# abiswas-odu/metagenomics

Hardware: NVIDIA B200
Metric: overlap_graph_build_reads_per_sec (higher is better)
Workload: dtype u64

## Files before the change

### include/ogb.h

```cpp
#ifndef OGB_H_
#define OGB_H_

#include <stddef.h>
#include <stdint.h>

#ifdef __cplusplus
extern "C" {
#endif

#define OGB_VERSION 210

enum {
	OGB_OK = 0,
	OGB_E_ARG = 1,
	OGB_E_CUDA = 2,
	OGB_E_NCCL = 3,
	OGB_E_STATE = 4,
	OGB_E_CAPACITY = 5,
	OGB_E_IO = 6,
	OGB_E_NOMEM = 7
};

typedef struct ogb_dataset ogb_dataset;
typedef struct ogb_context ogb_context;

typedef struct ogb_edge {
	uint32_t src;
	uint32_t dst;
	uint16_t offset;
	uint8_t orient;
	uint8_t reserved;
} ogb_edge;

enum {
	OGB_KC_HASH = 0,
	OGB_KC_WINDOW,
	OGB_KC_PROBE,
	OGB_KC_VERIFY,
	OGB_KC_ROWS,
	OGB_KC_MARK1,
	OGB_KC_MARK2,
	OGB_KC_MARKANY,
	OGB_KC_KEEP,
	OGB_KC_EMIT,
	OGB_KC_CONTAIN_WINDOW,
	OGB_KC_CONTAIN_PROBE,
	OGB_KC_CONTAIN_VERIFY,
	OGB_KC_EXCH_INDEX,
	OGB_KC_EXCH_ROWS,
	OGB_KC_EXCH_BITS,
	OGB_KC_EXCH_FINAL,
	OGB_KC_PROBE_VERIFY,
	OGB_KC_COUNT = 20
};

typedef struct ogb_stats {
	uint64_t n_reads;
	uint64_t table_buckets;
	uint64_t table_bytes;
	uint64_t n_contained;
	uint64_t contain_probes;
	uint64_t contain_hits;
	uint64_t overlap_probes;
	uint64_t probe_sectors;
	uint64_t candidates;
	uint64_t edges_pre;
	uint64_t edges_pre_local;
	uint64_t pivot_entries;
	uint64_t active_pivots;
	uint64_t edges_final;
	uint64_t nodes_final;
	uint64_t max_degree;
	uint64_t overflow_reads;
	uint32_t kernel_launches;
	uint32_t probe_launches;
	uint32_t hash_partitions;
	uint32_t hash_build_attempts;
	float ms_pack;
	float ms_hash_build;
	float ms_contain;
	float ms_overlap;
	float ms_exchange_pre;
	float ms_mark;
	float ms_reduce;
	float ms_total;
	float ms_scan_kernel;
	float ms_probe_launch;
	float ms_window_launch;
	float ms_kernel[OGB_KC_COUNT];
	uint32_t n_kernel[OGB_KC_COUNT];
} ogb_stats;

int ogb_version(void);
const char *ogb_last_error(void);


int ogb_dataset_create(ogb_dataset **out);
void ogb_dataset_destroy(ogb_dataset *ds);

int ogb_dataset_add_reads(ogb_dataset *ds, const char *bases, const uint64_t *offsets, uint64_t n);

int ogb_dataset_add_file(ogb_dataset *ds, const char *path);

int ogb_dataset_finalize(ogb_dataset *ds, uint32_t min_overlap);

int ogb_dataset_finalize_device(ogb_dataset *ds, ogb_context *ctx, uint32_t min_overlap);

uint64_t ogb_dataset_n_reads(const ogb_dataset *ds);
uint64_t ogb_dataset_n_unique(const ogb_dataset *ds);
uint64_t ogb_dataset_shortest(const ogb_dataset *ds);
uint64_t ogb_dataset_longest(const ogb_dataset *ds);
uint32_t ogb_dataset_min_overlap(const ogb_dataset *ds);

const uint64_t *ogb_dataset_words(const ogb_dataset *ds, uint64_t *n_words);
const uint64_t *ogb_dataset_word_offsets(const ogb_dataset *ds);
const uint16_t *ogb_dataset_lengths(const ogb_dataset *ds);
const uint32_t *ogb_dataset_frequencies(const ogb_dataset *ds);

int ogb_dataset_get_read(const ogb_dataset *ds, uint64_t id, int strand, char *out, uint32_t cap, uint32_t *len);

int ogb_dataset_find_read(const ogb_dataset *ds, const char *bases, uint32_t len, uint64_t *id);


int ogb_context_create(ogb_context **out, int device);

int ogb_nccl_unique_id(void *out128);
int ogb_context_create_dist(ogb_context **out, int device, int rank, int n_ranks, const void *nccl_uid);
void ogb_context_destroy(ogb_context *ctx);
int ogb_context_rank(const ogb_context *ctx, int *rank, int *n_ranks);

int ogb_reads_upload(ogb_context *ctx, const char *bases, const uint64_t *offsets, uint64_t n);
int ogb_reads_upload_packed(ogb_context *ctx, const uint64_t *words, const uint64_t *word_offsets,
                            const uint16_t *lengths, uint64_t n);
int ogb_reads_upload_dataset(ogb_context *ctx, const ogb_dataset *ds);
int ogb_reads_upload_packed_sharded(ogb_context *ctx, const uint64_t *shard_words, uint64_t n_total, uint32_t read_len);

int ogb_hash_build(ogb_context *ctx, uint32_t min_overlap);

int ogb_hash_lookup(ogb_context *ctx, const char *keys, uint64_t n_keys, uint64_t *out, uint64_t out_cap,
                    uint64_t *out_offsets);
uint64_t ogb_hash_string_length(const ogb_context *ctx);
uint64_t ogb_hash_table_size(const ogb_context *ctx);

int ogb_mark_contained(ogb_context *ctx);
int ogb_super_read_ids(ogb_context *ctx, uint64_t *out, uint64_t cap);

int ogb_mate_lookup(ogb_context *ctx, const char *bases, const uint64_t *offsets, uint64_t n_seqs, uint32_t min_overlap,
                    uint32_t *out_id, uint8_t *out_orient);

int ogb_build_graph(ogb_context *ctx, int keep_pre);

int ogb_graph_edge_count(ogb_context *ctx, int which, uint64_t *n);
int ogb_graph_edges(ogb_context *ctx, int which, ogb_edge *out, uint64_t cap);

int ogb_graph_edges_shard(ogb_context *ctx, ogb_edge *out, uint64_t cap, uint64_t *n_out);
int ogb_graph_checksum(ogb_context *ctx, int which, uint64_t *xor_out, uint64_t *sum_out);


typedef struct ogb_cedge {
	uint32_t src;
	uint32_t dst;
	uint64_t offset;
	uint64_t list_start;
	uint32_t count;
	uint32_t twin;
	uint8_t orient;
	uint8_t reserved[3];
	uint32_t reserved2;
} ogb_cedge;

typedef struct ogb_clist_item {
	uint32_t read;
	uint16_t offset;
	uint8_t orient;
	uint8_t reserved;
} ogb_clist_item;

typedef struct ogb_simplify_stats {
	uint64_t n_edges_in, n_edges_out, n_items;
	uint64_t merges, dead_ends;
	uint32_t iterations;
	uint32_t rounds;
	uint32_t jumps;
	uint32_t launches;
	float ms;
	float ms_setup;
	float ms_sweeps;
	float ms_dead_ends;
	float ms_lists;
	uint32_t reserved;
} ogb_simplify_stats;

int ogb_graph_simplify(ogb_context *ctx, ogb_simplify_stats *stats);
int ogb_graph_composite_edges(ogb_context *ctx, ogb_cedge *edges, uint64_t edge_cap, ogb_clist_item *items, uint64_t item_cap);


typedef struct ogb_unitig {
	uint32_t edge;
	uint32_t src;
	uint32_t dst;
	uint8_t orient;
	uint8_t reserved[3];
	uint64_t length;
	uint64_t start;
} ogb_unitig;

typedef struct ogb_spell_stats {
	uint64_t unitigs;
	uint64_t bases;
	uint64_t words;
	uint32_t launches;
	float ms;
} ogb_spell_stats;

int ogb_graph_spell(ogb_context *ctx, int canonical_only, uint64_t first, uint64_t count, ogb_spell_stats *stats);
int ogb_graph_unitigs(ogb_context *ctx, ogb_unitig *recs, uint64_t rec_cap, void *out, uint64_t out_cap, int ascii);
int ogb_graph_write_unitigs(ogb_context *ctx, const char *path);

int ogb_get_stats(ogb_context *ctx, ogb_stats *out);

int ogb_timer_begin(ogb_context *ctx);
int ogb_timer_end(ogb_context *ctx, float *ms);
int ogb_l2_flush(ogb_context *ctx, size_t bytes);

int ogb_gather_ceiling(ogb_context *ctx, size_t buffer_bytes, uint32_t gather_bytes, double *gb_per_s);

int ogb_alloc_host(void **out, size_t bytes);
void ogb_free_host(void *p);


int ogb_synth_genome(uint64_t seed, uint64_t len, char *out);

int ogb_synth_reads(uint64_t seed, const char *genomes, const uint64_t *g_offsets, const double *weights,
                    uint32_t n_genomes, uint64_t n_reads, uint32_t len_min, uint32_t len_max, int paired,
                    double insert_mean, double insert_sd, char *out_bases, uint64_t out_cap,
                    uint64_t *out_offsets);

#ifdef __cplusplus
}
#endif
#endif
```

### metagenomics_b200/_lib.py

```python
import ctypes as C
import os

_HERE = os.path.dirname(os.path.abspath(__file__))
LIB_PATH = os.environ.get("OGB_LIB") or os.path.join(_HERE, "libogb.so")

OGB_OK, OGB_E_ARG, OGB_E_CUDA, OGB_E_NCCL, OGB_E_STATE, OGB_E_CAPACITY, OGB_E_IO, OGB_E_NOMEM = range(8)


class OgbError(RuntimeError):
    def __init__(self, code, msg):
        super().__init__(f"libogb error {code}: {msg}")
        self.code = code


class Edge(C.Structure):
    _fields_ = [("src", C.c_uint32), ("dst", C.c_uint32), ("offset", C.c_uint16), ("orient", C.c_uint8),
                ("reserved", C.c_uint8)]


class Stats(C.Structure):
    _fields_ = [(n, C.c_uint64) for n in (
        "n_reads", "table_buckets", "table_bytes", "n_contained", "contain_probes", "contain_hits",
        "overlap_probes", "probe_sectors", "candidates", "edges_pre", "edges_pre_local", "pivot_entries",
        "active_pivots", "edges_final", "nodes_final", "max_degree", "overflow_reads")] + [
        ("kernel_launches", C.c_uint32), ("probe_launches", C.c_uint32), ("hash_partitions", C.c_uint32), ("hash_build_attempts", C.c_uint32)] + [(n, C.c_float) for n in (
            "ms_pack", "ms_hash_build", "ms_contain", "ms_overlap", "ms_exchange_pre", "ms_mark", "ms_reduce",
            "ms_total", "ms_scan_kernel", "ms_probe_launch", "ms_window_launch")] + [
        ("ms_kernel", C.c_float * 20), ("n_kernel", C.c_uint32 * 20)]

    KERNEL_CLASSES = ("hash_insert", "window_part", "probe_parts", "verify", "rows_finish", "mark_fast1", "mark_fast2", "mark_any", "keep", "emit",
                      "contain_window", "contain_probe", "contain_verify", "exch_index", "exch_rows", "exch_bits", "exch_final", "probe_verify")

    def as_dict(self):
        d = {n: getattr(self, n) for n, _ in self._fields_ if n not in ("ms_kernel", "n_kernel")}
        d["kernels"] = {k: {"ms": float(self.ms_kernel[i]), "launches": int(self.n_kernel[i])} for i, k in enumerate(self.KERNEL_CLASSES) if self.n_kernel[i]}
        return d


class SimplifyStats(C.Structure):
    _fields_ = [(n, C.c_uint64) for n in ("n_edges_in", "n_edges_out", "n_items", "merges", "dead_ends")] + [
        (n, C.c_uint32) for n in ("iterations", "rounds", "jumps", "launches")] + [
        (n, C.c_float) for n in ("ms", "ms_setup", "ms_sweeps", "ms_dead_ends", "ms_lists")] + [("reserved", C.c_uint32)]

    def as_dict(self):
        return {n: getattr(self, n) for n, _ in self._fields_ if n != "reserved"}


class SpellStats(C.Structure):
    _fields_ = [(n, C.c_uint64) for n in ("unitigs", "bases", "words")] + [("launches", C.c_uint32), ("ms", C.c_float)]

    def as_dict(self):
        return {n: getattr(self, n) for n, _ in self._fields_}


_u64p = C.POINTER(C.c_uint64)
_vp = C.c_void_p
PROTOTYPES = {
    "ogb_version": (C.c_int, []),
    "ogb_last_error": (C.c_char_p, []),
    "ogb_dataset_create": (C.c_int, [C.POINTER(_vp)]),
    "ogb_dataset_destroy": (None, [_vp]),
    "ogb_dataset_add_reads": (C.c_int, [_vp, _vp, _vp, C.c_uint64]),
    "ogb_dataset_add_file": (C.c_int, [_vp, C.c_char_p]),
    "ogb_dataset_finalize": (C.c_int, [_vp, C.c_uint32]),
    "ogb_dataset_finalize_device": (C.c_int, [_vp, _vp, C.c_uint32]),
    "ogb_dataset_n_reads": (C.c_uint64, [_vp]),
    "ogb_dataset_n_unique": (C.c_uint64, [_vp]),
    "ogb_dataset_shortest": (C.c_uint64, [_vp]),
    "ogb_dataset_longest": (C.c_uint64, [_vp]),
    "ogb_dataset_min_overlap": (C.c_uint32, [_vp]),
    "ogb_dataset_words": (_vp, [_vp, _u64p]),
    "ogb_dataset_word_offsets": (_vp, [_vp]),
    "ogb_dataset_lengths": (_vp, [_vp]),
    "ogb_dataset_frequencies": (_vp, [_vp]),
    "ogb_dataset_get_read": (C.c_int, [_vp, C.c_uint64, C.c_int, _vp, C.c_uint32, C.POINTER(C.c_uint32)]),
    "ogb_dataset_find_read": (C.c_int, [_vp, C.c_char_p, C.c_uint32, _u64p]),
    "ogb_context_create": (C.c_int, [C.POINTER(_vp), C.c_int]),
    "ogb_nccl_unique_id": (C.c_int, [_vp]),
    "ogb_context_create_dist": (C.c_int, [C.POINTER(_vp), C.c_int, C.c_int, C.c_int, _vp]),
    "ogb_context_destroy": (None, [_vp]),
    "ogb_context_rank": (C.c_int, [_vp, C.POINTER(C.c_int), C.POINTER(C.c_int)]),
    "ogb_reads_upload": (C.c_int, [_vp, _vp, _vp, C.c_uint64]),
    "ogb_reads_upload_packed": (C.c_int, [_vp, _vp, _vp, _vp, C.c_uint64]),
    "ogb_reads_upload_dataset": (C.c_int, [_vp, _vp]),
    "ogb_reads_upload_packed_sharded": (C.c_int, [_vp, _vp, C.c_uint64, C.c_uint32]),
    "ogb_hash_build": (C.c_int, [_vp, C.c_uint32]),
    "ogb_hash_lookup": (C.c_int, [_vp, _vp, C.c_uint64, _vp, C.c_uint64, _vp]),
    "ogb_hash_string_length": (C.c_uint64, [_vp]),
    "ogb_hash_table_size": (C.c_uint64, [_vp]),
    "ogb_mark_contained": (C.c_int, [_vp]),
    "ogb_super_read_ids": (C.c_int, [_vp, _vp, C.c_uint64]),
    "ogb_mate_lookup": (C.c_int, [_vp, _vp, _vp, C.c_uint64, C.c_uint32, _vp, _vp]),
    "ogb_build_graph": (C.c_int, [_vp, C.c_int]),
    "ogb_graph_edge_count": (C.c_int, [_vp, C.c_int, _u64p]),
    "ogb_graph_edges": (C.c_int, [_vp, C.c_int, _vp, C.c_uint64]),
    "ogb_graph_edges_shard": (C.c_int, [_vp, _vp, C.c_uint64, _u64p]),
    "ogb_graph_checksum": (C.c_int, [_vp, C.c_int, _u64p, _u64p]),
    "ogb_graph_simplify": (C.c_int, [_vp, C.POINTER(SimplifyStats)]),
    "ogb_graph_composite_edges": (C.c_int, [_vp, _vp, C.c_uint64, _vp, C.c_uint64]),
    "ogb_graph_spell": (C.c_int, [_vp, C.c_int, C.c_uint64, C.c_uint64, C.POINTER(SpellStats)]),
    "ogb_graph_unitigs": (C.c_int, [_vp, _vp, C.c_uint64, _vp, C.c_uint64, C.c_int]),
    "ogb_graph_write_unitigs": (C.c_int, [_vp, C.c_char_p]),
    "ogb_get_stats": (C.c_int, [_vp, C.POINTER(Stats)]),
    "ogb_timer_begin": (C.c_int, [_vp]),
    "ogb_timer_end": (C.c_int, [_vp, C.POINTER(C.c_float)]),
    "ogb_l2_flush": (C.c_int, [_vp, C.c_size_t]),
    "ogb_gather_ceiling": (C.c_int, [_vp, C.c_size_t, C.c_uint32, C.POINTER(C.c_double)]),
    "ogb_alloc_host": (C.c_int, [C.POINTER(_vp), C.c_size_t]),
    "ogb_free_host": (None, [_vp]),
    "ogb_synth_genome": (C.c_int, [C.c_uint64, C.c_uint64, _vp]),
    "ogb_synth_reads": (C.c_int, [C.c_uint64, _vp, _vp, _vp, C.c_uint32, C.c_uint64, C.c_uint32, C.c_uint32, C.c_int,
                                  C.c_double, C.c_double, _vp, C.c_uint64, _vp]),
}

_lib = None


def lib():
    global _lib
    if _lib is None:
        if not os.path.exists(LIB_PATH):
            raise OgbError(-1, f"{LIB_PATH} is missing: run `python -c 'import __graft_entry__ as g; g.build()'` "
                               "(there is no CPU fallback)")
        l = C.CDLL(LIB_PATH, mode=C.RTLD_GLOBAL)
        for name, (res, args) in PROTOTYPES.items():
            f = getattr(l, name)
            f.restype, f.argtypes = res, args
        _lib = l
    return _lib


def check(rc):
    if rc != OGB_OK:
        raise OgbError(rc, lib().ogb_last_error().decode("utf-8", "replace"))
```

### metagenomics_b200/csrc/ogb_device.cu

```cuda

#include "ogb_internal.h"
#include "ogb_kernels.cuh"
#include "ogb_contract.cuh"
#include "ogb_spell.cuh"

#include <algorithm>
#include <chrono>
#include <cstdio>
#include <cstring>
#include <dlfcn.h>
#include <string>
#include <vector>

#define CUDA_TRY(x)                                                                                      \
	do {                                                                                                 \
		cudaError_t e_ = (x);                                                                            \
		if (e_ != cudaSuccess) {                                                                         \
			ogb_set_error("CUDA error %s at %s:%d (%s)", cudaGetErrorString(e_), __FILE__, __LINE__, #x); \
			return OGB_E_CUDA;                                                                           \
		}                                                                                                \
	} while (0)
#define OGB_TRY(x) do { int r_ = (x); if (r_ != OGB_OK) return r_; } while (0)

typedef struct ncclComm *ncclComm_t;
typedef struct { char internal[128]; } ncclUniqueId;
enum { NCCL_UINT8 = 1, NCCL_UINT32 = 3, NCCL_UINT64 = 5 };
enum { NCCL_MAX = 2 };
struct NcclApi {
	void *lib = nullptr;
	int (*GetUniqueId)(ncclUniqueId *) = nullptr;
	int (*CommInitRank)(ncclComm_t *, int, ncclUniqueId, int) = nullptr;
	int (*CommDestroy)(ncclComm_t) = nullptr;
	int (*AllGather)(const void *, void *, size_t, int, ncclComm_t, cudaStream_t) = nullptr;
	int (*AllReduce)(const void *, void *, size_t, int, int, ncclComm_t, cudaStream_t) = nullptr;
	int (*Broadcast)(const void *, void *, size_t, int, int, ncclComm_t, cudaStream_t) = nullptr;
	int (*Send)(const void *, size_t, int, int, ncclComm_t, cudaStream_t) = nullptr;
	int (*Recv)(void *, size_t, int, int, ncclComm_t, cudaStream_t) = nullptr;
	int (*GroupStart)() = nullptr;
	int (*GroupEnd)() = nullptr;
	const char *(*GetErrorString)(int) = nullptr;
};
static NcclApi g_nccl;
static int nccl_load()
{
	if (g_nccl.lib) return OGB_OK;
	void *lib = dlopen("libnccl.so.2", RTLD_NOW | RTLD_GLOBAL);
	if (!lib) lib = dlopen("libnccl.so", RTLD_NOW | RTLD_GLOBAL);
	if (!lib) { ogb_set_error("cannot load libnccl.so.2: %s", dlerror()); return OGB_E_NCCL; }
#define SYM(field, name) *(void **)(&g_nccl.field) = dlsym(lib, name); if (!g_nccl.field) { ogb_set_error("libnccl: missing %s", name); return OGB_E_NCCL; }
	SYM(GetUniqueId, "ncclGetUniqueId") SYM(CommInitRank, "ncclCommInitRank") SYM(CommDestroy, "ncclCommDestroy")
	SYM(AllGather, "ncclAllGather") SYM(AllReduce, "ncclAllReduce") SYM(Broadcast, "ncclBroadcast") SYM(Send, "ncclSend") SYM(Recv, "ncclRecv")
	SYM(GroupStart, "ncclGroupStart") SYM(GroupEnd, "ncclGroupEnd") SYM(GetErrorString, "ncclGetErrorString")
#undef SYM
	g_nccl.lib = lib;
	return OGB_OK;
}
#define NCCL_TRY(x)                                                                                   \
	do {                                                                                              \
		int r_ = (x);                                                                                 \
		if (r_ != 0) { ogb_set_error("NCCL error %s at %s:%d", g_nccl.GetErrorString(r_), __FILE__, __LINE__); return OGB_E_NCCL; } \
	} while (0)

template <class T> struct Pool {
	T *p = nullptr;
	size_t cap = 0;
	int ensure(size_t need)
	{
		if (need <= cap) return OGB_OK;
		if (p) cudaFree(p);
		p = nullptr; cap = 0;
		cudaError_t e = cudaMalloc((void **)&p, need * sizeof(T));
		if (e != cudaSuccess) { ogb_set_error("cudaMalloc of %zu bytes failed: %s", need * sizeof(T), cudaGetErrorString(e)); return OGB_E_NOMEM; }
		cap = need;
		return OGB_OK;
	}
	void release() { if (p) cudaFree(p); p = nullptr; cap = 0; }
};

enum { OGB_MAX_RANKS = 64, XCHG_PER_RANK = 8, XCHG_SCRATCH = XCHG_PER_RANK * OGB_MAX_RANKS, XCHG_WORDS = XCHG_SCRATCH + 8 };


template <class T> struct Tmp {
	T *p = nullptr;
	cudaStream_t st = nullptr;
	int ensure(size_t need, cudaStream_t stream)
	{
		if (p) return OGB_OK;
		st = stream;
		cudaError_t e = cudaMallocAsync((void **)&p, std::max<size_t>(need, 1) * sizeof(T), stream);
		if (e != cudaSuccess) { ogb_set_error("cudaMallocAsync of %zu bytes failed: %s", need * sizeof(T), cudaGetErrorString(e)); p = nullptr; return OGB_E_NOMEM; }
		return OGB_OK;
	}
	void release() { if (p) cudaFreeAsync(p, st); p = nullptr; }
};

enum { EV_BEGIN = 0, EV_PACK0, EV_PACK1, EV_HASH0, EV_HASH1, EV_CONT0, EV_CONT1, EV_OVL0, EV_OVL1, EV_XPRE1, EV_MARK1, EV_RED1, EV_K3A, EV_K3B, EV_T0, EV_T1, EV_COUNT };

struct ogb_context {
	int device = 0, rank = 0, nranks = 1, sm_count = 148;
	cudaStream_t stream = nullptr;
	cudaStream_t stream2 = nullptr;
	cudaEvent_t ev_probe[2] = {}, ev_verify[2] = {};
	cudaEvent_t ev_pk[2 * 64] = {};
	cudaEvent_t ev_pm[64] = {};
	u32 n_pk = 0;
	struct KEv { cudaEvent_t a = nullptr, b = nullptr; int cls = 0; };
	std::vector<KEv> kev;
	u32 n_kev = 0;
	ncclComm_t comm = nullptr;
	cudaEvent_t ev[EV_COUNT] = {};
	Pool<u64> words, meta;
	Pool<u64> ds_words;
	ogb_dataset *pending_ds = nullptr;
	Pool<char> stage_bytes;
	Pool<u64> stage_offs;
	Pool<unsigned short> stage_lens;
	u32 n = 0, uniform_len = 0, uniform_pw = 0, min_len = 0, max_len = 0;
	bool have_reads = false;
	uint64_t reads_stamp = 0;
	Pool<u32> slots, summary;
	u32 nb = 0, h = 0, nparts = 1;
	bool use_summary = false;
	bool have_table = false;
	Pool<u64> sup;
	Pool<u32> contained;
	bool contain_done = false, any_contained = false;
	Pool<u64> pos, sums, surv;
	Pool<u64> cand, big;
	Pool<u32> cnt, cntc, scratch_keys;
	Pool<ogb_edge> fin, pre, fin_stage;
	Pool<u64> slots_e, ext;
	Pool<u32> deg;
	Pool<u32> rows, more, more_own, ebits, hrows;
	u64 more_stride = 0, more_cap = 0;
	cudaStream_t xs = nullptr;
	u32 *peer_rows[64] = {};
	const void *rows_shared = nullptr;
	bool rows_dma = false;
	cudaEvent_t ev_rows[2] = {}, ev_xs = nullptr;
	Pool<u32> cand_q, fill, ov_q;
	Pool<u64> cand_v, ov_e;
	u64 cand_cap = 0;
	Pool<u32> pq_b, pq_f, pq_q;
	u64 *d_pq_cursor = nullptr;
	bool partitioned = false, part_chunk_set = false;
	u64 pq_cap = 0;
	u32 pq_slack = 5;
	u64 *d_cursor = nullptr;
	u64 *d_xchg = nullptr;
	u32 slot_cap = 64;
	u32 chunk_reads = 1u << 16;
	int probe_blocks_per_sm = 0, verify_blocks_per_sm = 0;
	Pool<char> flush;
	u64 n_final = 0, n_pre = 0;
	u64 fin_own_off = 0, fin_own_cnt = 0;
	bool have_graph = false, have_pre = false;
	u64 *d_ctr = nullptr, *h_ctr = nullptr;
	u64 *d_tot = nullptr;
	Pool<CEntry> sE;
	Pool<CRec> s_rec;
	Pool<u32> s_rowptr, s_cp, s_info, s_list, s_keep, s_items, s_blocker;
	Pool<uint8_t> s_state, s_ready, s_flag;
	Pool<u64> s_epos, s_lpos, s_ctr;
	Pool<ogb_cedge> s_out;
	Pool<ogb_clist_item> s_out_items;
	bool have_simplified = false;
	uint64_t s_stamp = 0;
	ogb_simplify_stats sst = {};
	Pool<u32> sp_sel, sp_ioff, sp_nw;
	Pool<u64> sp_rank, sp_ipos, sp_wpos, sp_words;
	Pool<ogb_unitig> sp_rec;
	Pool<char> sp_ascii;
	bool have_spelled = false;
	u64 sp_first = 0;
	ogb_spell_stats spst = {};
	const void *l2_window_ptr = nullptr;
	size_t l2_window_bytes = 0;
	bool l2_refused = false;
	ogb_stats st = {};
	u32 launches = 0;

	ReadStore rs() const { ReadStore r; r.words = words.p; r.meta = uniform_len ? nullptr : meta.p; r.n = n; r.uniform_len = uniform_len; r.uniform_pw = uniform_pw; return r; }
	Table tb() const
	{
		Table t;
		t.slots = slots.p; t.summary = use_summary ? summary.p : nullptr; t.nb = nb; t.nparts = nparts; t.part_buckets = nb / nparts;
		t.sub = nparts / nranks; t.my_rank = rank; t.h = h; t.ctr = d_ctr;
		return t;
	}
	void shard(u32 &lo, u32 &hi) const
	{
		u64 per = ((u64)n + nranks - 1) / nranks;
		lo = (u32)std::min<u64>(n, per * rank);
		hi = (u32)std::min<u64>(n, per * (rank + 1));
	}
};

enum { OGB_KEV_MAX = 4096 };
static int kev_begin(ogb_context *c, int cls, cudaStream_t st)
{
	if (c->n_kev >= OGB_KEV_MAX) return -1;
	if (c->n_kev >= c->kev.size()) {
		ogb_context::KEv e;
		if (cudaEventCreate(&e.a) != cudaSuccess || cudaEventCreate(&e.b) != cudaSuccess) { cudaGetLastError(); return -1; }
		c->kev.push_back(e);
	}
	const int i = (int)c->n_kev++;
	c->kev[i].cls = cls;
	cudaEventRecord(c->kev[i].a, st);
	return i;
}
static void kev_end(ogb_context *c, int i, cudaStream_t st) { if (i >= 0) cudaEventRecord(c->kev[i].b, st); }
static void kev_collect(ogb_context *c)
{
	for (u32 i = 0; i < c->n_kev; i++) {
		float ms = 0;
		if (cudaEventElapsedTime(&ms, c->kev[i].a, c->kev[i].b) == cudaSuccess) { c->st.ms_kernel[c->kev[i].cls] += ms; c->st.n_kernel[c->kev[i].cls]++; }
		else cudaGetLastError();
	}
	c->n_kev = 0;
}
#define KEV(cls, stream, launch) do { const int kev_i_ = kev_begin(c, cls, stream); launch; kev_end(c, kev_i_, stream); } while (0)

static int fetch_words_cb(ogb_dataset *ds);

static int ctr_zero(ogb_context *c) { CUDA_TRY(cudaMemsetAsync(c->d_ctr, 0, CTR_COUNT * sizeof(u64), c->stream)); return OGB_OK; }
static int ctr_fetch(ogb_context *c)
{
	CUDA_TRY(cudaMemcpyAsync(c->h_ctr, c->d_ctr, CTR_COUNT * sizeof(u64), cudaMemcpyDeviceToHost, c->stream));
	CUDA_TRY(cudaStreamSynchronize(c->stream));
	return OGB_OK;
}
static int grid_for(ogb_context *c, const void *kernel, int block)
{
	int per_sm = 1;
	if (cudaOccupancyMaxActiveBlocksPerMultiprocessor(&per_sm, kernel, block, 0) != cudaSuccess || per_sm < 1) per_sm = 1;
	return c->sm_count * per_sm;
}
static float ev_ms(ogb_context *c, int a, int b) { float ms = 0; if (cudaEventElapsedTime(&ms, c->ev[a], c->ev[b]) != cudaSuccess) { cudaGetLastError(); return 0; } return ms; }

static int context_create_common(ogb_context **out, int device)
{
	if (!out) { ogb_set_error("ogb_context_create: out is NULL"); return OGB_E_ARG; }
	*out = nullptr;
	int count = 0;
	cudaError_t e = cudaGetDeviceCount(&count);
	if (e != cudaSuccess || count == 0) {
		ogb_set_error("no usable CUDA device (%s); libogb has no CPU fallback", e != cudaSuccess ? cudaGetErrorString(e) : "device count 0");
		cudaGetLastError();
		return OGB_E_CUDA;
	}
	if (device < 0 || device >= count) { ogb_set_error("device %d out of range (%d devices)", device, count); return OGB_E_ARG; }
	CUDA_TRY(cudaSetDevice(device));
	ogb_context *c = new ogb_context();
	c->device = device;
	cudaDeviceProp prop;
	CUDA_TRY(cudaGetDeviceProperties(&prop, device));
	c->sm_count = prop.multiProcessorCount;
	{
		const char *g = getenv("OGB_L2_FETCH");
		size_t gran = g ? (size_t)atoi(g) : 0;
		if (gran == 32 || gran == 64 || gran == 128) cudaDeviceSetLimit(cudaLimitMaxL2FetchGranularity, gran);
		cudaGetLastError();
	}
	CUDA_TRY(cudaStreamCreateWithFlags(&c->stream, cudaStreamNonBlocking));
	{
		cudaMemPool_t pool;
		if (cudaDeviceGetDefaultMemPool(&pool, device) == cudaSuccess) { uint64_t keep = 2ull << 30; cudaMemPoolSetAttribute(pool, cudaMemPoolAttrReleaseThreshold, &keep); }
		cudaGetLastError();
	}
	for (int i = 0; i < EV_COUNT; i++) CUDA_TRY(cudaEventCreate(&c->ev[i]));
	for (int i = 0; i < 128; i++) CUDA_TRY(cudaEventCreate(&c->ev_pk[i]));
	for (int i = 0; i < 64; i++) CUDA_TRY(cudaEventCreate(&c->ev_pm[i]));
	CUDA_TRY(cudaMalloc((void **)&c->d_ctr, CTR_COUNT * sizeof(u64)));
	CUDA_TRY(cudaMalloc((void **)&c->d_tot, 2 * sizeof(u64)));
	CUDA_TRY(cudaMalloc((void **)&c->d_cursor, 2 * sizeof(u64)));
	CUDA_TRY(cudaMalloc((void **)&c->d_pq_cursor, OGB_MAXPART * sizeof(u64)));
	CUDA_TRY(cudaMalloc((void **)&c->d_xchg, XCHG_WORDS * sizeof(u64)));
	CUDA_TRY(cudaMemset(c->d_xchg, 0, XCHG_WORDS * sizeof(u64)));
	CUDA_TRY(cudaStreamCreateWithFlags(&c->stream2, cudaStreamNonBlocking));
	CUDA_TRY(cudaStreamCreateWithFlags(&c->xs, cudaStreamNonBlocking));
	for (int i = 0; i < 2; i++) CUDA_TRY(cudaEventCreateWithFlags(&c->ev_rows[i], cudaEventDisableTiming));
	CUDA_TRY(cudaEventCreateWithFlags(&c->ev_xs, cudaEventDisableTiming));
	for (int i = 0; i < 2; i++) { CUDA_TRY(cudaEventCreateWithFlags(&c->ev_probe[i], cudaEventDisableTiming)); CUDA_TRY(cudaEventCreateWithFlags(&c->ev_verify[i], cudaEventDisableTiming)); }
	CUDA_TRY(cudaMemset(c->d_tot, 0, 2 * sizeof(u64)));
	CUDA_TRY(cudaMallocHost((void **)&c->h_ctr, CTR_COUNT * sizeof(u64)));
	CUDA_TRY(cudaMemset(c->d_ctr, 0, CTR_COUNT * sizeof(u64)));
	*out = c;
	return OGB_OK;
}

extern "C" int ogb_context_create(ogb_context **out, int device) { return context_create_common(out, device); }

extern "C" int ogb_nccl_unique_id(void *out128)
{
	if (!out128) { ogb_set_error("ogb_nccl_unique_id: NULL output"); return OGB_E_ARG; }
	OGB_TRY(nccl_load());
	ncclUniqueId id;
	NCCL_TRY(g_nccl.GetUniqueId(&id));
	memcpy(out128, &id, sizeof id);
	return OGB_OK;
}

extern "C" int ogb_context_create_dist(ogb_context **out, int device, int rank, int n_ranks, const void *nccl_uid)
{
	if (n_ranks < 1 || rank < 0 || rank >= n_ranks) { ogb_set_error("ogb_context_create_dist: bad rank %d of %d", rank, n_ranks); return OGB_E_ARG; }
	if (n_ranks > OGB_MAX_RANKS || n_ranks > OGB_MAXPART) { ogb_set_error("ogb_context_create_dist: at most %d ranks", OGB_MAX_RANKS < OGB_MAXPART ? OGB_MAX_RANKS : OGB_MAXPART); return OGB_E_ARG; }
	OGB_TRY(context_create_common(out, device));
	ogb_context *c = *out;
	c->rank = rank; c->nranks = n_ranks;
	if (n_ranks > 1) {
		if (!nccl_uid) { ogb_set_error("ogb_context_create_dist: NULL nccl id"); return OGB_E_ARG; }
		OGB_TRY(nccl_load());
		ncclUniqueId id;
		memcpy(&id, nccl_uid, sizeof id);
		NCCL_TRY(g_nccl.CommInitRank(&c->comm, n_ranks, id, rank));
	}
	return OGB_OK;
}

extern "C" void ogb_context_destroy(ogb_context *c)
{
	if (!c) return;
	cudaSetDevice(c->device);
	cudaStreamSynchronize(c->stream);
	if (c->pending_ds) fetch_words_cb(c->pending_ds);
	if (c->l2_window_ptr) cudaCtxResetPersistingL2Cache();
	if (c->stream2) cudaStreamSynchronize(c->stream2);
	if (c->xs) cudaStreamSynchronize(c->xs);
	{
		bool mapped = false;
		for (int p = 0; p < 64; p++) if (c->peer_rows[p]) { cudaIpcCloseMemHandle(c->peer_rows[p]); c->peer_rows[p] = nullptr; mapped = true; }
		if (mapped && c->comm) {
			g_nccl.AllReduce(c->d_xchg + XCHG_SCRATCH + 6, c->d_xchg + XCHG_SCRATCH + 6, 1, NCCL_UINT64, 2 , c->comm, c->stream);
			cudaStreamSynchronize(c->stream);
		}
	}
	if (c->comm) g_nccl.CommDestroy(c->comm);
	c->words.release(); c->meta.release(); c->ds_words.release(); c->stage_bytes.release(); c->stage_offs.release(); c->stage_lens.release();
	c->slots.release(); c->summary.release(); c->sup.release(); c->contained.release(); c->pos.release();
	c->sums.release(); c->surv.release(); c->cand.release(); c->big.release(); c->cntc.release(); c->cnt.release();
	c->scratch_keys.release(); c->fin.release(); c->pre.release(); c->flush.release(); c->fin_stage.release();
	c->sE.release(); c->s_rec.release(); c->s_rowptr.release(); c->s_cp.release(); c->s_info.release(); c->s_list.release(); c->s_keep.release(); c->s_items.release(); c->s_blocker.release();
	c->s_state.release(); c->s_ready.release(); c->s_flag.release(); c->s_epos.release(); c->s_lpos.release(); c->s_ctr.release(); c->s_out.release(); c->s_out_items.release();
	c->sp_sel.release(); c->sp_ioff.release(); c->sp_nw.release(); c->sp_rank.release(); c->sp_ipos.release(); c->sp_wpos.release(); c->sp_words.release();
	c->sp_rec.release(); c->sp_ascii.release();
	if (c->d_ctr) cudaFree(c->d_ctr);
	if (c->d_tot) cudaFree(c->d_tot);
	if (c->d_cursor) cudaFree(c->d_cursor);
	if (c->d_pq_cursor) cudaFree(c->d_pq_cursor);
	c->pq_b.release(); c->pq_f.release(); c->pq_q.release();
	if (c->d_xchg) cudaFree(c->d_xchg);
	c->cand_q.release(); c->deg.release(); c->fill.release(); c->ov_q.release();
	c->cand_v.release(); c->slots_e.release(); c->ext.release(); c->ov_e.release(); c->rows.release(); c->more.release(); c->more_own.release(); c->hrows.release(); c->ebits.release();
	if (c->h_ctr) cudaFreeHost(c->h_ctr);
	for (int i = 0; i < EV_COUNT; i++) if (c->ev[i]) cudaEventDestroy(c->ev[i]);
	for (int i = 0; i < 128; i++) if (c->ev_pk[i]) cudaEventDestroy(c->ev_pk[i]);
	for (int i = 0; i < 64; i++) if (c->ev_pm[i]) cudaEventDestroy(c->ev_pm[i]);
	for (auto &e : c->kev) { if (e.a) cudaEventDestroy(e.a); if (e.b) cudaEventDestroy(e.b); }
	for (int i = 0; i < 2; i++) { if (c->ev_probe[i]) cudaEventDestroy(c->ev_probe[i]); if (c->ev_verify[i]) cudaEventDestroy(c->ev_verify[i]); }
	for (int i = 0; i < 2; i++) if (c->ev_rows[i]) cudaEventDestroy(c->ev_rows[i]);
	if (c->ev_xs) cudaEventDestroy(c->ev_xs);
	if (c->xs) cudaStreamDestroy(c->xs);
	if (c->stream2) cudaStreamDestroy(c->stream2);
	if (c->stream) cudaStreamDestroy(c->stream);
	delete c;
}

extern "C" int ogb_context_rank(const ogb_context *c, int *rank, int *n_ranks)
{
	if (!c) { ogb_set_error("NULL context"); return OGB_E_ARG; }
	if (rank) *rank = c->rank;
	if (n_ranks) *n_ranks = c->nranks;
	return OGB_OK;
}

extern "C" int ogb_alloc_host(void **out, size_t bytes)
{
	if (!out) { ogb_set_error("ogb_alloc_host: NULL output"); return OGB_E_ARG; }
	cudaError_t e = cudaMallocHost(out, bytes ? bytes : 1);
	if (e != cudaSuccess) { ogb_set_error("cudaMallocHost(%zu) failed: %s", bytes, cudaGetErrorString(e)); cudaGetLastError(); return OGB_E_CUDA; }
	return OGB_OK;
}
extern "C" void ogb_free_host(void *p) { if (p) cudaFreeHost(p); }


static int layout_reads(ogb_context *c, const std::vector<u32> &lens, u64 &total_words, std::vector<u64> &meta_host)
{
	u32 n = (u32)lens.size();
	u32 mn = 0xFFFFFFFFu, mx = 0;
	for (u32 i = 0; i < n; i++) { mn = std::min(mn, lens[i]); mx = std::max(mx, lens[i]); }
	c->n = n; c->min_len = n ? mn : 0; c->max_len = mx;
	if (n && mn == mx) {
		c->uniform_len = mx;
		c->uniform_pw = ((mx + 63) >> 6) << 1;
		total_words = (u64)n * 2 * c->uniform_pw;
		meta_host.clear();
	} else {
		c->uniform_len = 0; c->uniform_pw = 0;
		meta_host.resize(n);
		u64 off = 0;
		for (u32 i = 0; i < n; i++) {
			if (off >= (1ull << 47)) { ogb_set_error("read store too large"); return OGB_E_CAPACITY; }
			meta_host[i] = (off << 16) | lens[i];
			off += 2 * (u64)(((lens[i] + 63) >> 6) << 1);
		}
		total_words = off;
	}
	return OGB_OK;
}

static int upload_common(ogb_context *c, u64 total_words, const std::vector<u64> &meta_host)
{
	OGB_TRY(c->words.ensure(total_words + 8));
	CUDA_TRY(cudaMemsetAsync(c->words.p + total_words, 0, 8 * sizeof(u64), c->stream));
	if (!meta_host.empty()) {
		OGB_TRY(c->meta.ensure(meta_host.size()));
		CUDA_TRY(cudaMemcpyAsync(c->meta.p, meta_host.data(), meta_host.size() * sizeof(u64), cudaMemcpyHostToDevice, c->stream));
	}
	c->slot_cap = 64;
	c->reads_stamp++;
	c->have_reads = true; c->have_table = false; c->contain_done = false; c->any_contained = false; c->have_graph = false; c->have_pre = false; c->have_spelled = false;
	return OGB_OK;
}

extern "C" int ogb_reads_upload(ogb_context *c, const char *bases, const uint64_t *offsets, uint64_t n)
{
	if (!c || (n && (!bases || !offsets))) { ogb_set_error("ogb_reads_upload: NULL argument"); return OGB_E_ARG; }
	if (n >= (1ull << 30)) { ogb_set_error("ogb_reads_upload: at most 2^30-1 reads per context"); return OGB_E_CAPACITY; }
	CUDA_TRY(cudaSetDevice(c->device));
	std::vector<u32> lens(n);
	for (u64 i = 0; i < n; i++) {
		u64 L = offsets[i + 1] - offsets[i];
		if (L < 2 || L > 65535) { ogb_set_error("ogb_reads_upload: read %llu has length %llu (allowed 2..65535)", (unsigned long long)(i + 1), (unsigned long long)L); return OGB_E_ARG; }
		lens[i] = (u32)L;
	}
	u64 total_words = 0;
	std::vector<u64> meta_host;
	OGB_TRY(layout_reads(c, lens, total_words, meta_host));
	OGB_TRY(upload_common(c, total_words, meta_host));
	if (n == 0) return OGB_OK;
	u64 nbytes = offsets[n] - offsets[0];
	OGB_TRY(c->stage_bytes.ensure(nbytes));
	OGB_TRY(c->stage_offs.ensure(n + 1));
	std::vector<u64> rel(n + 1);
	for (u64 i = 0; i <= n; i++) rel[i] = offsets[i] - offsets[0];
	CUDA_TRY(cudaEventRecord(c->ev[EV_PACK0], c->stream));
	CUDA_TRY(cudaMemcpyAsync(c->stage_bytes.p, bases + offsets[0], nbytes, cudaMemcpyHostToDevice, c->stream));
	CUDA_TRY(cudaMemcpyAsync(c->stage_offs.p, rel.data(), (n + 1) * sizeof(u64), cudaMemcpyHostToDevice, c->stream));
	u32 max_pw = ((c->max_len + 63) >> 6) << 1;
	u64 threads = (u64)n * max_pw;
	k_pack_ascii<<<(unsigned)((threads + 255) / 256), 256, 0, c->stream>>>(c->stage_bytes.p, c->stage_offs.p, c->words.p,
	                                                                      c->uniform_len ? nullptr : c->meta.p, (u32)n, c->uniform_len, c->uniform_pw, max_pw);
	CUDA_TRY(cudaGetLastError());
	CUDA_TRY(cudaEventRecord(c->ev[EV_PACK1], c->stream));
	CUDA_TRY(cudaStreamSynchronize(c->stream));
	c->st.ms_pack = ev_ms(c, EV_PACK0, EV_PACK1);
	c->st.n_reads = n;
	return OGB_OK;
}

extern "C" int ogb_reads_upload_packed(ogb_context *c, const uint64_t *words, const uint64_t *word_offsets, const uint16_t *lengths, uint64_t n)
{
	if (!c || (n && (!words || !word_offsets || !lengths))) { ogb_set_error("ogb_reads_upload_packed: NULL argument"); return OGB_E_ARG; }
	if (n >= (1ull << 30)) { ogb_set_error("ogb_reads_upload_packed: at most 2^30-1 reads per context"); return OGB_E_CAPACITY; }
	CUDA_TRY(cudaSetDevice(c->device));
	uint16_t mn = 0xFFFF, mx = 0;
	for (u64 i = 0; i < n; i++) { mn = std::min(mn, lengths[i]); mx = std::max(mx, lengths[i]); }
	if (n && mn < 2) { ogb_set_error("ogb_reads_upload_packed: a read is shorter than 2"); return OGB_E_ARG; }
	u64 total_words = 0;
	std::vector<u64> meta_host;
	const u64 in_words = n ? word_offsets[n] - word_offsets[0] : 0;
	const bool regular = n && mn == mx && in_words == n * (u64)((mx + 31) / 32);
	if (regular) {
		c->n = (u32)n; c->min_len = c->max_len = mx; c->uniform_len = mx; c->uniform_pw = ((mx + 63) >> 6) << 1;
		total_words = n * 2 * c->uniform_pw;
	} else {
		std::vector<u32> lens(n);
		for (u64 i = 0; i < n; i++) lens[i] = lengths[i];
		OGB_TRY(layout_reads(c, lens, total_words, meta_host));
	}
	OGB_TRY(upload_common(c, total_words, meta_host));
	if (n == 0) return OGB_OK;
	OGB_TRY(c->stage_bytes.ensure(in_words * sizeof(u64)));
	std::vector<u64> rel;
	const u64 *offs_src = (const u64 *)word_offsets;
	if (!regular) {
		OGB_TRY(c->stage_offs.ensure(n + 1));
		OGB_TRY(c->stage_lens.ensure(n));
		if (word_offsets[0] != 0) { rel.resize(n + 1); for (u64 i = 0; i <= n; i++) rel[i] = word_offsets[i] - word_offsets[0]; offs_src = rel.data(); }
	}
	CUDA_TRY(cudaEventRecord(c->ev[EV_PACK0], c->stream));
	CUDA_TRY(cudaMemcpyAsync(c->stage_bytes.p, words + word_offsets[0], in_words * sizeof(u64), cudaMemcpyHostToDevice, c->stream));
	if (!regular) {
		CUDA_TRY(cudaMemcpyAsync(c->stage_offs.p, offs_src, (n + 1) * sizeof(u64), cudaMemcpyHostToDevice, c->stream));
		CUDA_TRY(cudaMemcpyAsync(c->stage_lens.p, lengths, n * sizeof(uint16_t), cudaMemcpyHostToDevice, c->stream));
	}
	u32 max_pw = ((c->max_len + 63) >> 6) << 1;
	u64 threads = (u64)n * max_pw;
	k_pack_words<<<(unsigned)((threads + 255) / 256), 256, 0, c->stream>>>((const u64 *)c->stage_bytes.p, regular ? nullptr : c->stage_offs.p,
	                                                                      regular ? nullptr : c->stage_lens.p, c->words.p,
	                                                                      c->uniform_len ? nullptr : c->meta.p, (u32)n, c->uniform_len, c->uniform_pw, max_pw);
	CUDA_TRY(cudaGetLastError());
	CUDA_TRY(cudaEventRecord(c->ev[EV_PACK1], c->stream));
	CUDA_TRY(cudaStreamSynchronize(c->stream));
	c->st.ms_pack = ev_ms(c, EV_PACK0, EV_PACK1);
	c->st.n_reads = n;
	return OGB_OK;
}

extern "C" int ogb_reads_upload_dataset(ogb_context *c, const ogb_dataset *ds)
{
	if (!c || !ds) { ogb_set_error("ogb_reads_upload_dataset: NULL argument"); return OGB_E_ARG; }
	if (ds->resident_ctx == c && ds->resident_stamp == c->reads_stamp && c->have_reads) return OGB_OK;
	uint64_t nw = 0;
	const uint64_t *w = ogb_dataset_words(ds, &nw);
	return ogb_reads_upload_packed(c, w, ogb_dataset_word_offsets(ds), ogb_dataset_lengths(ds), ogb_dataset_n_unique(ds));
}

extern "C" int ogb_reads_upload_packed_sharded(ogb_context *c, const uint64_t *shard_words, uint64_t n_total, uint32_t read_len)
{
	if (!c || (n_total && !shard_words)) { ogb_set_error("ogb_reads_upload_packed_sharded: NULL argument"); return OGB_E_ARG; }
	if (n_total >= (1ull << 30)) { ogb_set_error("ogb_reads_upload_packed_sharded: at most 2^30-1 reads per context"); return OGB_E_CAPACITY; }
	if (read_len < 2 || read_len > 65535) { ogb_set_error("ogb_reads_upload_packed_sharded: read length %u (allowed 2..65535)", read_len); return OGB_E_ARG; }
	CUDA_TRY(cudaSetDevice(c->device));
	const int G = c->nranks;
	c->n = (u32)n_total; c->min_len = c->max_len = read_len; c->uniform_len = read_len; c->uniform_pw = ((read_len + 63) >> 6) << 1;
	const u64 per = (n_total + G - 1) / G, stride = 2ull * c->uniform_pw, nw = (read_len + 31) / 32;
	const u64 total_words = per * G * stride;
	std::vector<u64> none;
	OGB_TRY(upload_common(c, total_words, none));
	if (n_total == 0) return OGB_OK;
	u32 lo, hi;
	c->shard(lo, hi);
	const u64 nloc = hi - lo;
	OGB_TRY(c->stage_bytes.ensure(std::max<u64>(nloc * nw, 1) * sizeof(u64)));
	CUDA_TRY(cudaEventRecord(c->ev[EV_PACK0], c->stream));
	if (nloc) {
		CUDA_TRY(cudaMemcpyAsync(c->stage_bytes.p, shard_words, nloc * nw * sizeof(u64), cudaMemcpyHostToDevice, c->stream));
		const u64 threads = nloc * c->uniform_pw;
		k_pack_words<<<(unsigned)((threads + 255) / 256), 256, 0, c->stream>>>((const u64 *)c->stage_bytes.p, nullptr, nullptr, c->words.p + (u64)lo * stride, nullptr,
		                                                                      (u32)nloc, c->uniform_len, c->uniform_pw, c->uniform_pw);
		CUDA_TRY(cudaGetLastError());
	}
	if (G > 1) NCCL_TRY(g_nccl.AllGather(c->words.p + per * stride * c->rank, c->words.p, per * stride, NCCL_UINT64, c->comm, c->stream));
	CUDA_TRY(cudaEventRecord(c->ev[EV_PACK1], c->stream));
	CUDA_TRY(cudaStreamSynchronize(c->stream));
	c->st.ms_pack = ev_ms(c, EV_PACK0, EV_PACK1);
	c->st.n_reads = n_total;
	return OGB_OK;
}

static int exclusive_scan(ogb_context *c, const u32 *cnt, u32 n, u64 *out, u64 *d_total, u64 *d_max = nullptr, u64 *d_more = nullptr);

static int fetch_words_cb(ogb_dataset *ds)
{
	ogb_context *c = (ogb_context *)ds->fetch_ctx;
	ds->fetch = nullptr; ds->fetch_ctx = nullptr;
	if (!c) return OGB_OK;
	if (c->pending_ds == ds) c->pending_ds = nullptr;
	CUDA_TRY(cudaSetDevice(c->device));
	ds->words.resize(ds->pending_words);
	if (ds->pending_words) {
		CUDA_TRY(cudaMemcpyAsync(ds->words.data(), c->ds_words.p, ds->pending_words * sizeof(u64), cudaMemcpyDeviceToHost, c->stream));
		CUDA_TRY(cudaStreamSynchronize(c->stream));
	}
	ds->pending_words = 0;
// ... 227 lines not shown
		c->partitioned = e ? atoi(e) != 0 : true;
	}
	c->launches = 0;
	c->n_kev = 0;
	memset(c->st.ms_kernel, 0, sizeof c->st.ms_kernel); memset(c->st.n_kernel, 0, sizeof c->st.n_kernel);
	CUDA_TRY(cudaEventRecord(c->ev[EV_HASH0], c->stream));
	u64 sub_limit = OGB_MAXPART / c->nranks, nb = 0;
	bool k1_direct = false;
	for (int attempt = 0;; attempt++) {
		if (attempt == 12) { ogb_set_error("ogb_hash_build: a hash partition kept filling up (%u partitions, %.1f buckets per read)", c->nparts, buckets_per_read); return OGB_E_CAPACITY; }
		nb = std::max<u64>((u64)(buckets_per_read * c->n) + 1, 512);
		{
			const u64 slice_bytes = nb * OGB_BWORDS * sizeof(u32) / c->nranks;
			u64 sub = slice_bytes > (192ull << 20) ? (slice_bytes + (160ull << 20) - 1) / (160ull << 20) : 1;
			const char *e = getenv("OGB_SUB_PARTITIONS");
			if (e && atoi(e) >= 1) sub = (u64)atoi(e);
			sub = std::max<u64>(1, std::min<u64>(sub, sub_limit));
			c->nparts = (u32)(c->nranks * sub);
		}
		nb = (nb + c->nparts - 1) / c->nparts * c->nparts;
		if (nb >= (1ull << 32)) { ogb_set_error("index too large"); return OGB_E_CAPACITY; }
		c->nb = (u32)nb;
		OGB_TRY(c->slots.ensure(nb * OGB_BWORDS));
		if (c->use_summary) OGB_TRY(c->summary.ensure(nb));
		{
			const u64 pb = nb / c->nranks;
			CUDA_TRY(cudaMemsetAsync(c->slots.p + pb * OGB_BWORDS * c->rank, 0, pb * OGB_BWORDS * sizeof(u32), c->stream));
			if (c->use_summary) CUDA_TRY(cudaMemsetAsync(c->summary.p + pb * c->rank, 0, pb * sizeof(u32), c->stream));
		}
		CUDA_TRY(cudaMemsetAsync(c->d_ctr + CTR_TABLE_FULL, 0, sizeof(u64), c->stream));
		if (c->n) {
			u64 threads = (u64)c->n * 4;
			const u32 sub = c->nparts / c->nranks;
			const char *eq = getenv("OGB_K1_QUEUES");
			const bool queued = sub > 1 && !k1_direct && !(eq && atoi(eq) == 0);
			if (queued) {
				const u64 qcap = threads / c->nparts * 5 / 4 + 4096;
				OGB_TRY(c->pq_b.ensure(qcap * sub)); OGB_TRY(c->pq_f.ensure(qcap * sub)); OGB_TRY(c->pq_q.ensure(qcap * sub));
				KeyQueue kq;
				kq.b = c->pq_b.p; kq.f = c->pq_f.p; kq.v = c->pq_q.p; kq.cursor = c->d_pq_cursor; kq.cap = qcap;
				kq.nparts = c->nparts; kq.first = (u32)c->rank * sub; kq.count = sub;
				CUDA_TRY(cudaMemsetAsync(c->d_pq_cursor, 0, OGB_MAXPART * sizeof(u64), c->stream));
				const u64 tiles = (threads + 256 * OGB_KPT - 1) / (256 * OGB_KPT);
				const int ke = kev_begin(c, OGB_KC_HASH, c->stream);
				k_key_part<<<(unsigned)std::min<u64>(grid_for(c, (const void *)k_key_part, 256), tiles), 256, 0, c->stream>>>(c->rs(), c->tb(), kq);
				k_insert_parts<<<grid_for(c, (const void *)k_insert_parts, 256), 256, 0, c->stream>>>(c->tb(), kq);
				kev_end(c, ke, c->stream);
				CUDA_TRY(cudaGetLastError());
				c->launches += 2;
			}
			if (!queued) {
				KEV(OGB_KC_HASH, c->stream, (k_hash_insert<<<(unsigned)((threads + 255) / 256), 256, 0, c->stream>>>(c->rs(), c->tb())));
				CUDA_TRY(cudaGetLastError());
				c->launches++;
			}
		}
		u64 full = 0;
		if (c->nranks > 1) NCCL_TRY(g_nccl.AllReduce(c->d_ctr + CTR_TABLE_FULL, c->d_ctr + CTR_TABLE_FULL, 1, NCCL_UINT64, NCCL_MAX, c->comm, c->stream));
		CUDA_TRY(cudaMemcpyAsync(c->h_ctr + CTR_TABLE_FULL, c->d_ctr + CTR_TABLE_FULL, sizeof(u64), cudaMemcpyDeviceToHost, c->stream));
		if (c->nranks > 1) {
			const u64 pb = nb / c->nranks;
			const int ke = kev_begin(c, OGB_KC_EXCH_INDEX, c->stream);
			NCCL_TRY(g_nccl.AllGather(c->slots.p + pb * OGB_BWORDS * c->rank, c->slots.p, pb * OGB_BWORDS, NCCL_UINT32, c->comm, c->stream));
			if (c->use_summary) NCCL_TRY(g_nccl.AllGather(c->summary.p + pb * c->rank, c->summary.p, pb, NCCL_UINT32, c->comm, c->stream));
			kev_end(c, ke, c->stream);
		}
		CUDA_TRY(cudaEventRecord(c->ev[EV_HASH1], c->stream));
		CUDA_TRY(cudaStreamSynchronize(c->stream));
		kev_collect(c);
		full = c->h_ctr[CTR_TABLE_FULL];
		c->st.hash_build_attempts = (uint32_t)attempt + 1;
		if (!full) break;
		if (full >= 2 && !k1_direct) { k1_direct = true; continue; }
		if (c->nparts > (u32)c->nranks) sub_limit = std::max<u64>(1, c->nparts / c->nranks / 2);
		else buckets_per_read *= 2;
	}
	OGB_TRY(l2_keep_summary(c, true));
	c->st.ms_hash_build = ev_ms(c, EV_HASH0, EV_HASH1);
	c->st.table_buckets = nb;
	c->st.hash_partitions = c->nparts;
	c->st.table_bytes = nb * OGB_BWORDS * sizeof(u32);
	c->part_chunk_set = false; c->pq_slack = 5;
	if (!c->partitioned && c->chunk_reads > (1u << 16)) c->chunk_reads = 1u << 16;
	c->have_table = true; c->contain_done = false; c->any_contained = false; c->have_graph = false;
	c->st.ms_contain = 0; c->st.n_contained = 0; c->st.contain_probes = 0; c->st.contain_hits = 0;
	return OGB_OK;
}

extern "C" uint64_t ogb_hash_string_length(const ogb_context *c) { return c ? c->h : 0; }
extern "C" uint64_t ogb_hash_table_size(const ogb_context *c) { return c ? (uint64_t)c->nb * OGB_SLOTS : 0; }

extern "C" int ogb_hash_lookup(ogb_context *c, const char *keys, uint64_t n_keys, uint64_t *out, uint64_t out_cap, uint64_t *out_offsets)
{
	if (!c || !out_offsets || (n_keys && !keys)) { ogb_set_error("ogb_hash_lookup: NULL argument"); return OGB_E_ARG; }
	if (!c->have_table) { ogb_set_error("ogb_hash_lookup: build the hash table first"); return OGB_E_STATE; }
	CUDA_TRY(cudaSetDevice(c->device));
	const u32 h = c->h, kw = (h + 31) / 32;
	out_offsets[0] = 0;
	if (n_keys == 0) return OGB_OK;
	std::vector<u64> packed(n_keys * (kw + 2) + 4, 0);
	for (u64 k = 0; k < n_keys; k++)
		for (u32 i = 0; i < h; i++) {
			u64 code;
			switch (keys[k * h + i]) {
			case 'A': case 'a': code = 0; break;
			case 'C': case 'c': code = 1; break;
			case 'G': case 'g': code = 2; break;
			case 'T': case 't': code = 3; break;
			default: ogb_set_error("ogb_hash_lookup: key %llu is not ACGT", (unsigned long long)k); return OGB_E_ARG;
			}
			packed[k * (kw + 2) + (i >> 5)] |= code << (62 - 2 * (i & 31));
		}
	Pool<u64> d_keys, d_pos, d_out;
	Pool<u32> d_cnt;
	int rc = OGB_OK;
	std::vector<u32> cnt(n_keys);
	std::vector<u64> pos(n_keys + 1, 0);
	auto run = [&]() -> int {
		OGB_TRY(d_keys.ensure(packed.size())); OGB_TRY(d_cnt.ensure(n_keys)); OGB_TRY(d_pos.ensure(n_keys + 1));
		CUDA_TRY(cudaMemcpyAsync(d_keys.p, packed.data(), packed.size() * sizeof(u64), cudaMemcpyHostToDevice, c->stream));
		unsigned grid = (unsigned)((n_keys + 127) / 128);
		k_lookup<<<grid, 128, 0, c->stream>>>(c->rs(), c->tb(), d_keys.p, kw, n_keys, d_cnt.p, nullptr, nullptr, 0);
		CUDA_TRY(cudaGetLastError());
		CUDA_TRY(cudaMemcpyAsync(cnt.data(), d_cnt.p, n_keys * sizeof(u32), cudaMemcpyDeviceToHost, c->stream));
		CUDA_TRY(cudaStreamSynchronize(c->stream));
		for (u64 k = 0; k < n_keys; k++) pos[k + 1] = pos[k] + cnt[k];
		for (u64 k = 0; k <= n_keys; k++) out_offsets[k] = pos[k];
		if (pos[n_keys] > out_cap || (pos[n_keys] && !out)) { ogb_set_error("ogb_hash_lookup: output needs %llu entries", (unsigned long long)pos[n_keys]); return OGB_E_CAPACITY; }
		if (pos[n_keys] == 0) return OGB_OK;
		OGB_TRY(d_out.ensure(pos[n_keys]));
		CUDA_TRY(cudaMemcpyAsync(d_pos.p, pos.data(), (n_keys + 1) * sizeof(u64), cudaMemcpyHostToDevice, c->stream));
		k_lookup<<<grid, 128, 0, c->stream>>>(c->rs(), c->tb(), d_keys.p, kw, n_keys, d_cnt.p, d_pos.p, d_out.p, 1);
		CUDA_TRY(cudaGetLastError());
		CUDA_TRY(cudaMemcpyAsync(out, d_out.p, pos[n_keys] * sizeof(u64), cudaMemcpyDeviceToHost, c->stream));
		CUDA_TRY(cudaStreamSynchronize(c->stream));
		for (u64 k = 0; k < n_keys; k++)
			std::sort(out + pos[k], out + pos[k + 1], [](u64 a, u64 b) {
				u64 ia = a & 0x3FFFFFFFFFFFFFFFull, ib = b & 0x3FFFFFFFFFFFFFFFull;
				return ia != ib ? ia < ib : (a >> 62) < (b >> 62);
			});
		return OGB_OK;
	};
	rc = run();
	d_keys.release(); d_pos.release(); d_out.release(); d_cnt.release();
	return rc;
}

static ScanArgs scan_args(ogb_context *c, u32 lo, u32 hi)
{
	ScanArgs a;
	a.R = c->rs(); a.T = c->tb(); a.lo = lo; a.hi = hi;
	a.contained = c->any_contained ? c->contained.p : nullptr;
	a.cand_q = c->cand_q.p; a.cand_v = c->cand_v.p; a.cand_cap = c->cand_cap; a.cand_cursor = c->d_cursor;
	a.sup = c->sup.p; a.slots_e = c->slots_e.p; a.slot_lo = lo; a.cap = c->slot_cap; a.deg = c->deg.p;
	a.ov_q = c->ov_q.p; a.ov_e = c->ov_e.p; a.ov_cap = c->ov_q.cap; a.ctr = c->d_ctr; a.prefetch = 1;
	return a;
}

static GraphView graph_view(const ogb_context *c, u32 lo);

static int share_rows(ogb_context *c)
{
	const int G = c->nranks;
	if (G == 1 || c->rows_shared == (const void *)c->rows.p) return OGB_OK;
	for (int p = 0; p < G; p++) if (c->peer_rows[p]) { cudaIpcCloseMemHandle(c->peer_rows[p]); c->peer_rows[p] = nullptr; }
	c->rows_dma = false;
	c->rows_shared = c->rows.p;
	const char *e = getenv("OGB_ROWS_NCCL");
	u64 ok = !(e && atoi(e) != 0);
	cudaIpcMemHandle_t mine;
	memset(&mine, 0, sizeof mine);
	if (ok && cudaIpcGetMemHandle(&mine, c->rows.p) != cudaSuccess) { cudaGetLastError(); ok = 0; }
	static_assert(sizeof(cudaIpcMemHandle_t) == 64, "IPC handle size");
	const size_t rec = 72;
	Pool<unsigned char> buf;
	OGB_TRY(buf.ensure(rec * G));
	std::vector<unsigned char> host(rec * G, 0);
	memcpy(host.data() + rec * c->rank, &mine, 64);
	memcpy(host.data() + rec * c->rank + 64, &ok, 8);
	CUDA_TRY(cudaMemcpyAsync(buf.p + rec * c->rank, host.data() + rec * c->rank, rec, cudaMemcpyHostToDevice, c->stream));
	NCCL_TRY(g_nccl.AllGather(buf.p + rec * c->rank, buf.p, rec, NCCL_UINT8, c->comm, c->stream));
	CUDA_TRY(cudaMemcpyAsync(host.data(), buf.p, rec * G, cudaMemcpyDeviceToHost, c->stream));
	CUDA_TRY(cudaStreamSynchronize(c->stream));
	buf.release();
	bool all = true;
	for (int p = 0; p < G; p++) { u64 f; memcpy(&f, host.data() + rec * p + 64, 8); all = all && f != 0; }
	u64 opened = all;
	if (all)
		for (int p = 0; p < G && opened; p++) {
			if (p == c->rank) continue;
			cudaIpcMemHandle_t h;
			memcpy(&h, host.data() + rec * p, 64);
			void *ptr = nullptr;
			if (cudaIpcOpenMemHandle(&ptr, h, cudaIpcMemLazyEnablePeerAccess) != cudaSuccess) { cudaGetLastError(); opened = 0; break; }
			c->peer_rows[p] = (u32 *)ptr;
		}
	CUDA_TRY(cudaMemcpyAsync(c->d_xchg + XCHG_SCRATCH + 6, &opened, sizeof(u64), cudaMemcpyHostToDevice, c->stream));
	NCCL_TRY(g_nccl.AllReduce(c->d_xchg + XCHG_SCRATCH + 6, c->d_xchg + XCHG_SCRATCH + 6, 1, NCCL_UINT64, 3 , c->comm, c->stream));
	CUDA_TRY(cudaMemcpyAsync(&opened, c->d_xchg + XCHG_SCRATCH + 6, sizeof(u64), cudaMemcpyDeviceToHost, c->stream));
	CUDA_TRY(cudaStreamSynchronize(c->stream));
	c->rows_dma = opened != 0;
	if (!c->rows_dma) for (int p = 0; p < G; p++) if (c->peer_rows[p]) { cudaIpcCloseMemHandle(c->peer_rows[p]); c->peer_rows[p] = nullptr; }
	return OGB_OK;
}

static int exchange_chunk_rows(ogb_context *c, u32 ci, cudaStream_t st)
{
	const int G = c->nranks;
	const u64 per = ((u64)c->n + G - 1) / G;
	auto range = [&](int r, u64 &a, u64 &b) {
		const u64 lo = std::min<u64>(c->n, per * r), hi = std::min<u64>(c->n, per * (r + 1));
		a = std::min(hi, lo + (u64)ci * c->chunk_reads); b = std::min(hi, a + c->chunk_reads);
	};
	u64 ma, mb;
	range(c->rank, ma, mb);
	if (c->rows_dma) {
		for (int k = 1; k < G && mb > ma; k++) {
			const int p = (c->rank + k) % G;
			CUDA_TRY(cudaMemcpyAsync(c->peer_rows[p] + ma * OGB_ROW_W, c->rows.p + ma * OGB_ROW_W, (mb - ma) * OGB_ROW_W * sizeof(u32), cudaMemcpyDeviceToDevice, st));
		}
		return OGB_OK;
	}
	NCCL_TRY(g_nccl.GroupStart());
	for (int p = 0; p < G; p++) {
		if (p == c->rank) continue;
		u64 pa, pb;
		range(p, pa, pb);
		if (mb > ma) NCCL_TRY(g_nccl.Send(c->rows.p + ma * OGB_ROW_W, (mb - ma) * OGB_ROW_W, NCCL_UINT32, p, c->comm, st));
		if (pb > pa) NCCL_TRY(g_nccl.Recv(c->rows.p + pa * OGB_ROW_W, (pb - pa) * OGB_ROW_W, NCCL_UINT32, p, c->comm, st));
	}
	NCCL_TRY(g_nccl.GroupEnd());
	return OGB_OK;
}

template <int MODE> static int scan_chunks(ogb_context *c, u32 lo, u32 hi)
{
	const bool part_mode = c->partitioned && hi > lo;
	const u32 nwin_u = (c->uniform_len ? c->uniform_len : c->max_len) - c->h - 1;
	{
		const char *e = getenv("OGB_CHUNK_READS");
		if (e && atoll(e) >= 256 && !part_mode) c->chunk_reads = (u32)std::min<long long>(atoll(e), 1ll << 16);
	}
	if (part_mode) {
		if (!c->part_chunk_set) { const char *e = getenv("OGB_CHUNK_READS"); c->chunk_reads = e && atoll(e) >= 256 ? (u32)std::min<long long>(atoll(e), 1ll << 23) : 3u << 17; c->part_chunk_set = true; }
		c->chunk_reads = (u32)std::max<u64>(256, std::min<u64>(c->chunk_reads, (64ull << 20) / std::max<u32>(nwin_u, 1)));
		const u64 pcap = std::min<u64>(c->chunk_reads, hi - lo) * nwin_u / c->nparts * std::min<u64>(c->pq_slack, 4ull * c->nparts) / 4 + 4096;
		OGB_TRY(c->pq_b.ensure(pcap * c->nparts)); OGB_TRY(c->pq_f.ensure(pcap * c->nparts)); OGB_TRY(c->pq_q.ensure(pcap * c->nparts));
		c->pq_cap = pcap;
	} else
	if (c->chunk_reads > (1u << 16)) c->chunk_reads = 1u << 16;
	{
		const u64 want = part_mode ? std::max<u64>(32ull << 20, (u64)c->chunk_reads * 40) : 8ull << 20;
		if (c->cand_cap < want) { OGB_TRY(c->cand_q.ensure(2 * want)); OGB_TRY(c->cand_v.ensure(2 * want)); c->cand_cap = want; }
	}
	int gp = grid_for(c, (const void *)k_probe<MODE>, 256), gv = grid_for(c, (const void *)k_verify<MODE>, 256);
	int gu = grid_for(c, (const void *)k_probe_uniform<MODE>, 256);
	{
		const char *ep = getenv("OGB_PROBE_BLOCKS_PER_SM"), *ev = getenv("OGB_VERIFY_BLOCKS_PER_SM");
		const int bp = ep ? atoi(ep) : c->probe_blocks_per_sm, bv = ev ? atoi(ev) : c->verify_blocks_per_sm;
		if (bp > 0) { gp = std::min(gp, c->sm_count * bp); gu = std::min(gu, c->sm_count * bp); }
		if (bv > 0) gv = std::min(gv, c->sm_count * bv);
	}
	const bool overlap_streams = getenv("OGB_ONE_STREAM") == nullptr;
	cudaStream_t sv = overlap_streams ? c->stream2 : c->stream;
	ScanArgs a = scan_args(c, lo, hi);
	u32 i = 0;
	const bool xchg = MODE == MODE_OVERLAP && c->nranks > 1;
	const u64 per_rank = ((u64)c->n + c->nranks - 1) / c->nranks;
	const u32 n_chunks = (u32)(((xchg ? per_rank : (u64)(hi - lo)) + c->chunk_reads - 1) / c->chunk_reads);
	const GraphView gv_rows = graph_view(c, lo);
	const int g_rows = grid_for(c, (const void *)k_rows_finish<false>, 256);
	const bool fused = part_mode && getenv("OGB_FUSED") && atoi(getenv("OGB_FUSED")) == 1;
	bool have_prev = false;
	ScanArgs a_prev = a;
	u32 prev_i = 0;
	auto finish_chunk = [&](const ScanArgs &av, u32 ci, cudaStream_t after) -> int {
		if (MODE != MODE_OVERLAP) return OGB_OK;
		CUDA_TRY(cudaEventRecord(c->ev_rows[ci & 1], after));
		CUDA_TRY(cudaStreamWaitEvent(c->xs, c->ev_rows[ci & 1], 0));
		KEV(OGB_KC_ROWS, c->xs, (k_rows_finish<false><<<std::min<int>(g_rows, (int)((av.hi - av.lo + 255) / 256)), 256, 0, c->xs>>>(gv_rows, av.lo, av.hi, c->more_own.p, c->more_cap, c->d_ctr, nullptr, 0)));
		c->launches++;
		if (xchg) {
			const int ke = kev_begin(c, OGB_KC_EXCH_ROWS, c->xs);
			OGB_TRY(exchange_chunk_rows(c, ci, c->xs));
			kev_end(c, ke, c->xs);
		}
		return OGB_OK;
	};
	auto flush_prev = [&]() -> int {
		if (!have_prev) return OGB_OK;
		KEV(MODE == MODE_OVERLAP ? OGB_KC_VERIFY : OGB_KC_CONTAIN_VERIFY, c->stream, (k_verify<MODE><<<gv, 256, 0, c->stream>>>(a_prev)));
		c->launches++;
		have_prev = false;
		return finish_chunk(a_prev, prev_i, c->stream);
	};
	for (; i < n_chunks; i++) {
		const u64 b0 = (u64)lo + (u64)i * c->chunk_reads;
		const int q = i & 1;
		if (b0 >= hi) {
			if (fused) OGB_TRY(flush_prev());
			if (xchg) { const int ke = kev_begin(c, OGB_KC_EXCH_ROWS, c->xs); OGB_TRY(exchange_chunk_rows(c, i, c->xs)); kev_end(c, ke, c->xs); }
			continue;
		}
		if (fused) {
			a.lo = (u32)b0; a.hi = (u32)std::min<u64>(hi, b0 + c->chunk_reads);
			a.cand_q = c->cand_q.p + q * c->cand_cap; a.cand_v = c->cand_v.p + q * c->cand_cap; a.cand_cursor = c->d_cursor + q;
			a.prefetch = 0;
			CUDA_TRY(cudaMemsetAsync(a.cand_cursor, 0, sizeof(u64), c->stream));
			CUDA_TRY(cudaMemsetAsync(c->d_pq_cursor, 0, OGB_MAXPART * sizeof(u64), c->stream));
			PartQueue pq;
			pq.b = c->pq_b.p; pq.f = c->pq_f.p; pq.q = c->pq_q.p; pq.cursor = c->d_pq_cursor; pq.cap = c->pq_cap; pq.nparts = c->nparts;
			const u32 nreads = a.hi - a.lo;
			const u64 tiles = ((u64)nreads * nwin_u + 256 * OGB_WPT - 1) / (256 * OGB_WPT);
			const bool uni = c->uniform_len && !a.contained;
			const int gw = grid_for(c, uni ? (const void *)k_window_part<MODE, true> : (const void *)k_window_part<MODE, false>, 256);
			const int kc = MODE == MODE_OVERLAP ? 0 : OGB_KC_CONTAIN_WINDOW - OGB_KC_WINDOW;
			const bool timed = MODE == MODE_OVERLAP && i < 64;
			if (timed) CUDA_TRY(cudaEventRecord(c->ev_pk[2 * i], c->stream));
			if (uni) KEV(OGB_KC_WINDOW + kc, c->stream, (k_window_part<MODE, true><<<(unsigned)std::min<u64>(gw, tiles), 256, 0, c->stream>>>(a, nwin_u, ~0ull / nwin_u + 1, pq)));
			else KEV(OGB_KC_WINDOW + kc, c->stream, (k_window_part<MODE, false><<<(unsigned)std::min<u64>(gw, tiles), 256, 0, c->stream>>>(a, nwin_u, ~0ull / nwin_u + 1, pq)));
			if (timed) CUDA_TRY(cudaEventRecord(c->ev_pm[i], c->stream));
			if (have_prev) {
				KEV(MODE == MODE_OVERLAP ? OGB_KC_PROBE_VERIFY : OGB_KC_CONTAIN_PROBE, c->stream,
				    (k_probe_verify<MODE><<<grid_for(c, (const void *)k_probe_verify<MODE>, 256), 256, 0, c->stream>>>(a, pq, a_prev)));
				OGB_TRY(finish_chunk(a_prev, prev_i, c->stream));
			} else
				KEV(OGB_KC_PROBE + kc, c->stream, (k_probe_parts<MODE><<<grid_for(c, (const void *)k_probe_parts<MODE>, 256), 256, 0, c->stream>>>(a, pq)));
			if (timed) { CUDA_TRY(cudaEventRecord(c->ev_pk[2 * i + 1], c->stream)); c->n_pk = i + 1; }
			c->launches += 2;
			have_prev = true; a_prev = a; prev_i = i;
			continue;
		}
		a.lo = (u32)b0; a.hi = (u32)std::min<u64>(hi, b0 + c->chunk_reads);
		a.cand_q = c->cand_q.p + q * c->cand_cap; a.cand_v = c->cand_v.p + q * c->cand_cap; a.cand_cursor = c->d_cursor + q;
		if (overlap_streams && i >= 2) CUDA_TRY(cudaStreamWaitEvent(c->stream, c->ev_verify[q], 0));
		CUDA_TRY(cudaMemsetAsync(a.cand_cursor, 0, sizeof(u64), c->stream));
		const u32 warps = a.hi - a.lo;
		const bool timed = MODE == MODE_OVERLAP && i < 64;
		if (timed) CUDA_TRY(cudaEventRecord(c->ev_pk[2 * i], c->stream));
		if (part_mode) {
			PartQueue pq;
			pq.b = c->pq_b.p; pq.f = c->pq_f.p; pq.q = c->pq_q.p; pq.cursor = c->d_pq_cursor; pq.cap = c->pq_cap; pq.nparts = c->nparts;
			a.prefetch = 0;
			CUDA_TRY(cudaMemsetAsync(c->d_pq_cursor, 0, OGB_MAXPART * sizeof(u64), c->stream));
			const u64 tiles = ((u64)warps * nwin_u + 256 * OGB_WPT - 1) / (256 * OGB_WPT);
			const bool uni = c->uniform_len && !a.contained;
			const int gw = grid_for(c, uni ? (const void *)k_window_part<MODE, true> : (const void *)k_window_part<MODE, false>, 256), gb = grid_for(c, (const void *)k_probe_parts<MODE>, 256);
			const int kc = MODE == MODE_OVERLAP ? 0 : OGB_KC_CONTAIN_WINDOW - OGB_KC_WINDOW;
			if (uni) KEV(OGB_KC_WINDOW + kc, c->stream, (k_window_part<MODE, true><<<(unsigned)std::min<u64>(gw, tiles), 256, 0, c->stream>>>(a, nwin_u, ~0ull / nwin_u + 1, pq)));
			else KEV(OGB_KC_WINDOW + kc, c->stream, (k_window_part<MODE, false><<<(unsigned)std::min<u64>(gw, tiles), 256, 0, c->stream>>>(a, nwin_u, ~0ull / nwin_u + 1, pq)));
			if (timed) CUDA_TRY(cudaEventRecord(c->ev_pm[i], c->stream));
			KEV(OGB_KC_PROBE + kc, c->stream, (k_probe_parts<MODE><<<gb, 256, 0, c->stream>>>(a, pq)));
			c->launches++;
		} else if (c->uniform_len && !a.contained) {
			const u32 nwin = c->uniform_len - c->h - 1;
			const u64 rounds = ((u64)warps * nwin + 31) / 32;
			KEV(MODE == MODE_OVERLAP ? OGB_KC_PROBE : OGB_KC_CONTAIN_PROBE, c->stream, (k_probe_uniform<MODE><<<(unsigned)std::min<u64>(gu, (rounds * 32 + 255) / 256), 256, 0, c->stream>>>(a, nwin, ~0ull / nwin + 1)));
		} else
			KEV(MODE == MODE_OVERLAP ? OGB_KC_PROBE : OGB_KC_CONTAIN_PROBE, c->stream, (k_probe<MODE><<<(unsigned)std::min<u64>(gp, ((u64)warps * 32 + 255) / 256), 256, 0, c->stream>>>(a)));
		if (timed) { CUDA_TRY(cudaEventRecord(c->ev_pk[2 * i + 1], c->stream)); c->n_pk = i + 1; }
		if (overlap_streams) {
			CUDA_TRY(cudaEventRecord(c->ev_probe[q], c->stream));
			CUDA_TRY(cudaStreamWaitEvent(sv, c->ev_probe[q], 0));
		}
		KEV(MODE == MODE_OVERLAP ? OGB_KC_VERIFY : OGB_KC_CONTAIN_VERIFY, sv, (k_verify<MODE><<<gv, 256, 0, sv>>>(a)));
		if (MODE == MODE_OVERLAP) {
			CUDA_TRY(cudaEventRecord(c->ev_rows[q], sv));
			CUDA_TRY(cudaStreamWaitEvent(c->xs, c->ev_rows[q], 0));
			KEV(OGB_KC_ROWS, c->xs, (k_rows_finish<false><<<std::min<int>(g_rows, (int)((a.hi - a.lo + 255) / 256)), 256, 0, c->xs>>>(gv_rows, a.lo, a.hi, c->more_own.p, c->more_cap, c->d_ctr, nullptr, 0)));
			c->launches++;
			if (xchg) {
				const int ke = kev_begin(c, OGB_KC_EXCH_ROWS, c->xs);
				OGB_TRY(exchange_chunk_rows(c, i, c->xs));
				kev_end(c, ke, c->xs);
			}
		}
		if (overlap_streams) CUDA_TRY(cudaEventRecord(c->ev_verify[q], sv));
		c->launches += 2;
	}
	if (fused) OGB_TRY(flush_prev());
	if (overlap_streams && !fused)
		for (int q = 0; q < 2 && q < (int)i; q++) CUDA_TRY(cudaStreamWaitEvent(c->stream, c->ev_verify[q], 0));
	if (MODE == MODE_OVERLAP) { CUDA_TRY(cudaEventRecord(c->ev_xs, c->xs)); CUDA_TRY(cudaStreamWaitEvent(c->stream, c->ev_xs, 0)); }
	CUDA_TRY(cudaGetLastError());
	return OGB_OK;
}

extern "C" int ogb_mark_contained(ogb_context *c)
{
	if (!c) { ogb_set_error("NULL context"); return OGB_E_ARG; }
	if (!c->have_table) { ogb_set_error("ogb_mark_contained: build the hash table first"); return OGB_E_STATE; }
	CUDA_TRY(cudaSetDevice(c->device));
	OGB_TRY(l2_keep_summary(c, true));
	c->contain_done = true; c->any_contained = false; c->have_graph = false;
	c->st.n_contained = 0; c->st.contain_probes = 0; c->st.contain_hits = 0; c->st.ms_contain = 0;
	OGB_TRY(c->sup.ensure((size_t)c->n + 1));
	CUDA_TRY(cudaMemsetAsync(c->sup.p, 0, ((size_t)c->n + 1) * sizeof(u64), c->stream));
	if (c->n == 0 || c->min_len == c->max_len) { CUDA_TRY(cudaStreamSynchronize(c->stream)); return OGB_OK; }
	OGB_TRY(c->contained.ensure(((size_t)c->n + 31) / 32 + 1));
	u32 lo, hi;
	c->shard(lo, hi);
	CUDA_TRY(cudaEventRecord(c->ev[EV_CONT0], c->stream));
	for (int attempt = 0;; attempt++) {
		if (attempt == 12) { ogb_set_error("ogb_mark_contained: candidate queue kept overflowing"); return OGB_E_CAPACITY; }
		OGB_TRY(ctr_zero(c));
		CUDA_TRY(cudaMemsetAsync(c->sup.p, 0, ((size_t)c->n + 1) * sizeof(u64), c->stream));
		bool saved = c->any_contained;
		c->any_contained = false;
		int rc = scan_chunks<MODE_CONTAIN>(c, lo, hi);
		c->any_contained = saved;
		OGB_TRY(rc);
		OGB_TRY(ctr_fetch(c));
		if (c->h_ctr[CTR_CAND_MAX] > c->cand_cap) { c->chunk_reads = std::max<u32>(256, c->chunk_reads / 2); continue; }
		break;
	}
	c->st.contain_probes = c->h_ctr[CTR_PROBES];
	c->st.contain_hits = c->h_ctr[CTR_CONTAIN_HITS];
	OGB_TRY(ctr_zero(c));
	if (c->nranks > 1) NCCL_TRY(g_nccl.AllReduce(c->sup.p, c->sup.p, c->n, NCCL_UINT64, NCCL_MAX, c->comm, c->stream));
	k_contained_bitmap<<<(c->n + 255) / 256, 256, 0, c->stream>>>(c->sup.p, c->n, c->contained.p, c->d_ctr);
	CUDA_TRY(cudaGetLastError());
	c->launches++;
	CUDA_TRY(cudaEventRecord(c->ev[EV_CONT1], c->stream));
	OGB_TRY(ctr_fetch(c));
	kev_collect(c);
	c->st.ms_contain = ev_ms(c, EV_CONT0, EV_CONT1);
	c->st.n_contained = c->h_ctr[CTR_N_CONTAINED];
	c->any_contained = c->st.n_contained > 0;
	return OGB_OK;
}

extern "C" int ogb_super_read_ids(ogb_context *c, uint64_t *out, uint64_t cap)
{
	if (!c || !out) { ogb_set_error("ogb_super_read_ids: NULL argument"); return OGB_E_ARG; }
	if (cap < (uint64_t)c->n + 1) { ogb_set_error("ogb_super_read_ids: need %u entries", c->n + 1); return OGB_E_CAPACITY; }
	out[0] = 0;
	if (!c->contain_done || c->n == 0) { for (u32 i = 1; i <= c->n; i++) out[i] = 0; return OGB_OK; }
	CUDA_TRY(cudaSetDevice(c->device));
	CUDA_TRY(cudaMemcpyAsync(out + 1, c->sup.p, (size_t)c->n * sizeof(u64), cudaMemcpyDeviceToHost, c->stream));
	CUDA_TRY(cudaStreamSynchronize(c->stream));
	for (u32 i = 1; i <= c->n; i++) out[i] = out[i] ? (uint64_t)(0xFFFFFFFFu - (u32)(out[i] & 0xFFFFFFFFull)) + 1 : 0;
	return OGB_OK;
}

static int exclusive_scan(ogb_context *c, const u32 *cnt, u32 n, u64 *out, u64 *d_total, u64 *d_max, u64 *d_more)
{
	u32 nblocks = (n + OGB_SCAN_ITEMS - 1) / OGB_SCAN_ITEMS;
	if (nblocks == 0) nblocks = 1;
	OGB_TRY(c->sums.ensure(nblocks + 1));
	k_scan_sums<<<nblocks, 256, 0, c->stream>>>(cnt, n, c->sums.p, d_max, d_more);
	k_scan_top<<<1, 1024, 0, c->stream>>>(c->sums.p, nblocks, d_total);
	k_scan_apply<<<nblocks, 256, 0, c->stream>>>(cnt, n, c->sums.p, out);
	CUDA_TRY(cudaGetLastError());
	c->launches += 3;
	return OGB_OK;
}

static GraphView graph_view(const ogb_context *c, u32 lo)
{
	GraphView g;
	const u64 per = ((u64)c->n + c->nranks - 1) / c->nranks;
	g.slots = c->slots_e.p; g.deg = c->deg.p; g.ext = c->ext.p; g.lo = lo; g.cap = c->slot_cap;
	g.rows = c->rows.p; g.more = c->nranks > 1 ? c->more.p : c->more_own.p; g.ebits = c->ebits.p;
	g.more_stride = c->more_stride; g.nrows = per * c->nranks;
	g.per_magic = c->nranks > 1 && per > 1 ? ~0ull / per + 1 : 0;
	g.my_rank = (u32)c->rank;
	return g;
}

template <class T> static int gather_segments(ogb_context *c, Pool<T> &stage, u64 stride, const std::vector<u64> &count, T *out)
{
	const int G = c->nranks;
	if (stride) NCCL_TRY(g_nccl.AllGather(stage.p + stride * c->rank, stage.p, stride * sizeof(T), NCCL_UINT8, c->comm, c->stream));
	u64 at = 0;
	for (int r = 0; r < G; r++) {
		if (count[r]) CUDA_TRY(cudaMemcpyAsync(out + at, stage.p + stride * r, count[r] * sizeof(T), cudaMemcpyDeviceToDevice, c->stream));
		at += count[r];
	}
	return OGB_OK;
}

extern "C" int ogb_build_graph(ogb_context *c, int keep_pre)
{
	if (!c) { ogb_set_error("NULL context"); return OGB_E_ARG; }
	if (!c->have_table) { ogb_set_error("ogb_build_graph: build the hash table first"); return OGB_E_STATE; }
	CUDA_TRY(cudaSetDevice(c->device));
	OGB_TRY(l2_keep_summary(c, true));
	if (!c->contain_done) OGB_TRY(ogb_mark_contained(c));
	c->have_graph = false; c->have_pre = false; c->have_simplified = false; c->have_spelled = false; c->n_final = 0; c->n_pre = 0;
	const u32 n = c->n;
	if (n == 0) { c->have_graph = true; c->have_pre = keep_pre != 0; c->st.edges_pre = c->st.edges_pre_local = c->st.edges_final = c->st.nodes_final = 0; return OGB_OK; }
	u32 lo, hi;
	c->shard(lo, hi);
	const int G = c->nranks;
	const u64 per = ((u64)n + G - 1) / G;
	const u32 nloc = hi - lo;
	{
		const char *e = getenv("OGB_SLOT_CAP");
		if (e && atoi(e) >= 8 && atoi(e) <= 256) c->slot_cap = (u32)atoi(e);
	}
	OGB_TRY(c->cnt.ensure(per + 1));
	OGB_TRY(c->cntc.ensure(per + 1));
	OGB_TRY(c->pos.ensure(per + 1));
	OGB_TRY(c->fill.ensure(per + 1));
	OGB_TRY(c->surv.ensure((per + 1) * OGB_SURV));
	OGB_TRY(c->cand.ensure((per + 1) * OGB_SURV * 2));
	if (G > 1 && per * G * OGB_ROW_W + 64 > c->rows.cap && c->rows_shared) {
		for (int p = 0; p < G; p++) if (c->peer_rows[p]) { cudaIpcCloseMemHandle(c->peer_rows[p]); c->peer_rows[p] = nullptr; }
		c->rows_dma = false; c->rows_shared = nullptr;
		NCCL_TRY(g_nccl.AllReduce(c->d_xchg + XCHG_SCRATCH + 6, c->d_xchg + XCHG_SCRATCH + 6, 1, NCCL_UINT64, 2 , c->comm, c->stream));
		CUDA_TRY(cudaStreamSynchronize(c->stream));
	}
	OGB_TRY(c->rows.ensure(per * G * OGB_ROW_W + 64));
	OGB_TRY(share_rows(c));
	if (c->ov_q.cap == 0) { OGB_TRY(c->ov_q.ensure(1 << 20)); OGB_TRY(c->ov_e.ensure(1 << 20)); }

	CUDA_TRY(cudaEventRecord(c->ev[EV_OVL0], c->stream));
	u64 local_edges = 0, exact_edges = 0, more_need = 0, heavy_max = 0;
	std::vector<u64> seg_cnt(G, 0), hrow_cnt(G, 0);
	for (int attempt = 0;; attempt++) {
		if (attempt == 16) { ogb_set_error("ogb_build_graph: staging pools kept overflowing"); return OGB_E_CAPACITY; }
		OGB_TRY(c->slots_e.ensure(per * c->slot_cap + 64));
		OGB_TRY(c->deg.ensure((size_t)n + 1));
		OGB_TRY(c->ext.ensure(1 << 16));
		if (c->more_cap == 0) c->more_cap = per * 8 + 1024;
		OGB_TRY(c->more_own.ensure((c->more_cap + 1023) & ~1023ull));
		OGB_TRY(ctr_zero(c));
		if (nloc) CUDA_TRY(cudaMemsetAsync(c->deg.p + lo, 0, (size_t)nloc * sizeof(u32), c->stream));
		CUDA_TRY(cudaEventRecord(c->ev[EV_K3A], c->stream));
		OGB_TRY(scan_chunks<MODE_OVERLAP>(c, lo, hi));
		CUDA_TRY(cudaEventRecord(c->ev[EV_K3B], c->stream));
		OGB_TRY(exclusive_scan(c, c->deg.p + lo, nloc, c->pos.p, c->d_tot, c->d_ctr + CTR_MAX_DEGREE, c->d_ctr + CTR_MORE_NEED));
		CUDA_TRY(cudaMemcpyAsync(&local_edges, c->d_tot, sizeof(u64), cudaMemcpyDeviceToHost, c->stream));
		OGB_TRY(ctr_fetch(c));
		const u64 n_over = c->h_ctr[CTR_OVERFLOW], n_heavy = c->h_ctr[CTR_BIG_NODES];
		u64 verdict[XCHG_PER_RANK] = {c->h_ctr[CTR_CAND_MAX] > c->cand_cap, n_over, c->h_ctr[CTR_MAX_DEGREE], local_edges, n_over + n_heavy * c->slot_cap, c->h_ctr[CTR_PQ_OVERFLOW] != 0, c->h_ctr[CTR_MORE_NEED], n_heavy};
		more_need = verdict[6]; heavy_max = n_heavy;
		seg_cnt[0] = local_edges; exact_edges = local_edges;
		hrow_cnt.assign(G, 0); hrow_cnt[0] = n_heavy;
		if (G > 1) {
			CUDA_TRY(cudaMemcpyAsync(c->d_xchg + XCHG_PER_RANK * c->rank, verdict, sizeof verdict, cudaMemcpyHostToDevice, c->stream));
			NCCL_TRY(g_nccl.AllGather(c->d_xchg + XCHG_PER_RANK * c->rank, c->d_xchg, XCHG_PER_RANK, NCCL_UINT64, c->comm, c->stream));
			std::vector<u64> all((size_t)XCHG_PER_RANK * G);
			CUDA_TRY(cudaMemcpyAsync(all.data(), c->d_xchg, all.size() * sizeof(u64), cudaMemcpyDeviceToHost, c->stream));
			CUDA_TRY(cudaStreamSynchronize(c->stream));
			exact_edges = 0;
			for (int r = 0; r < G; r++) {
				const u64 *v = &all[(size_t)XCHG_PER_RANK * r];
				verdict[0] = std::max(verdict[0], v[0]); verdict[1] = std::max(verdict[1], v[1]); verdict[2] = std::max(verdict[2], v[2]); verdict[5] = std::max(verdict[5], v[5]);
				more_need = std::max(more_need, v[6]); heavy_max = std::max(heavy_max, v[7]);
				seg_cnt[r] = v[3]; exact_edges += v[3]; hrow_cnt[r] = v[7];
			}
		}
		if (verdict[5]) { c->pq_slack *= 2; continue; }
		if (more_need > c->more_cap) { c->more_cap = more_need + more_need / 8 + 1024; continue; }
		if (verdict[0]) { c->chunk_reads = std::max<u32>(256, c->chunk_reads / 2); continue; }
		if (verdict[1] > c->ov_q.cap) {
			if (c->slot_cap < 256) c->slot_cap *= 2;
			else { OGB_TRY(c->ov_q.ensure(verdict[1] + verdict[1] / 8 + 1024)); OGB_TRY(c->ov_e.ensure(verdict[1] + verdict[1] / 8 + 1024)); }
			continue;
		}
		c->st.max_degree = verdict[2];
		c->st.overflow_reads = n_heavy;
		if (verdict[1]) {
			OGB_TRY(c->ext.ensure(n_over + n_heavy * c->slot_cap + 64));
			if (n_over) {
				k_heavy_move<<<(nloc + 255) / 256, 256, 0, c->stream>>>(c->slots_e.p, c->deg.p, lo, hi, c->slot_cap, c->ext.p, c->ext.cap, c->fill.p, c->d_ctr);
				k_heavy_place<<<(unsigned)((n_over + 255) / 256), 256, 0, c->stream>>>(c->ov_q.p, c->ov_e.p, n_over, c->slots_e.p, lo, c->slot_cap, c->ext.p, c->fill.p);
				CUDA_TRY(cudaGetLastError());
				c->launches += 2;
			}
		}
		break;
	}
	c->st.overlap_probes = c->h_ctr[CTR_PROBES];
	c->st.probe_sectors = c->h_ctr[CTR_SECTORS];
	c->st.candidates = c->h_ctr[CTR_CANDIDATES];
	c->st.edges_pre_local = local_edges;
	c->st.edges_pre = exact_edges;
	c->n_pre = exact_edges;
	CUDA_TRY(cudaEventRecord(c->ev[EV_OVL1], c->stream));
	OGB_TRY(l2_keep_summary(c, false));

	if (more_need >= (1ull << 32) - 2048) { ogb_set_error("ogb_build_graph: adjacency overflow area too large"); return OGB_E_CAPACITY; }
	c->more_stride = G > 1 ? std::max<u64>(1024, (more_need + 1023) & ~1023ull) : ((c->more_cap + 1023) & ~1023ull);
	if (G > 1) OGB_TRY(c->more.ensure(c->more_stride * G));
	const u64 nrows = per * G, obit_words = c->more_stride / 32;
	OGB_TRY(c->ebits.ensure(nrows + obit_words * G + 2));
	CUDA_TRY(cudaMemsetAsync(c->ebits.p + nrows + obit_words * c->rank, 0, obit_words * sizeof(u32), c->stream));
	if (heavy_max) {
		const u64 hstride = heavy_max;
		if (G > 1) OGB_TRY(c->hrows.ensure(hstride * G * OGB_HROW_W));
		u32 *my_h = G > 1 ? c->hrows.p + hstride * c->rank * OGB_HROW_W : nullptr;
		if (nloc && hrow_cnt[c->rank])
			KEV(OGB_KC_ROWS, c->stream, (k_rows_finish<true><<<grid_for(c, (const void *)k_rows_finish<true>, 256), 256, 0, c->stream>>>(graph_view(c, lo), lo, hi, c->more_own.p, c->more_cap, c->d_ctr, my_h, hstride)));
		CUDA_TRY(cudaGetLastError());
		c->launches++;
		if (G > 1) {
			const int ke = kev_begin(c, OGB_KC_EXCH_ROWS, c->stream);
			NCCL_TRY(g_nccl.AllGather(c->hrows.p + hstride * c->rank * OGB_HROW_W, c->hrows.p, hstride * OGB_HROW_W, NCCL_UINT32, c->comm, c->stream));
			kev_end(c, ke, c->stream);
			OGB_TRY(c->sums.ensure(G + 8));
			CUDA_TRY(cudaMemcpyAsync(c->sums.p, hrow_cnt.data(), (size_t)G * sizeof(u64), cudaMemcpyHostToDevice, c->stream));
			k_scatter_hrows<<<c->sm_count, 256, 0, c->stream>>>(c->hrows.p, hstride, c->sums.p, (u32)G, (u32)c->rank, c->rows.p);
			CUDA_TRY(cudaGetLastError());
			c->launches++;
		}
	}
	if (G > 1 && more_need) {
		const int ke = kev_begin(c, OGB_KC_EXCH_ROWS, c->stream);
		NCCL_TRY(g_nccl.AllGather(c->more_own.p, c->more.p, c->more_stride, NCCL_UINT32, c->comm, c->stream));
		kev_end(c, ke, c->stream);
	}
	CUDA_TRY(cudaEventRecord(c->ev[EV_XPRE1], c->stream));

	const u32 cap_now = c->slot_cap;
	const int g_emit = grid_for(c, (const void *)k_emit<false>, OGB_WARPS * 32);
	if (keep_pre) {
		OGB_TRY(c->pre.ensure(std::max<u64>(exact_edges, 1)));
		if (G == 1) {
			k_emit<true><<<g_emit, OGB_WARPS * 32, 0, c->stream>>>(c->slots_e.p, c->ext.p, c->deg.p, nullptr, c->pos.p, c->pre.p, lo, hi, cap_now, 0, 0);
			CUDA_TRY(cudaGetLastError());
		} else {
			u64 stride = 0;
			for (int r = 0; r < G; r++) stride = std::max(stride, seg_cnt[r]);
			stride = (stride + 63) & ~63ull;
			OGB_TRY(c->fin_stage.ensure(std::max<u64>(stride * G, 1)));
			k_emit<true><<<g_emit, OGB_WARPS * 32, 0, c->stream>>>(c->slots_e.p, c->ext.p, c->deg.p, nullptr, c->pos.p, c->fin_stage.p, lo, hi, cap_now, stride * c->rank, 0);
			CUDA_TRY(cudaGetLastError());
			OGB_TRY(gather_segments(c, c->fin_stage, stride, seg_cnt, c->pre.p));
		}
		c->have_pre = true;
	}

	MarkArgs m;
	m.G = graph_view(c, lo);
	m.hi = hi; m.cnt = c->cnt.p; m.cntc = c->cntc.p; m.cand = c->cand.p;
	OGB_TRY(c->big.ensure((local_edges + 1) * 3));
	m.big = c->big.p; m.big_cap = local_edges + 1;
	if (c->scratch_keys.cap == 0) OGB_TRY(c->scratch_keys.ensure(1 << 20));
	for (int attempt = 0;; attempt++) {
		if (attempt == 4) { ogb_set_error("ogb_build_graph: neighbour-set scratch kept overflowing"); return OGB_E_CAPACITY; }
		OGB_TRY(ctr_zero(c));
		m.scratch_keys = c->scratch_keys.p; m.scratch_cap = c->scratch_keys.cap; m.ctr = c->d_ctr;
		KEV(OGB_KC_MARK1, c->stream, (k_mark_fast<1><<<grid_for(c, (const void *)k_mark_fast<1>, OGB_WARPS * 32), OGB_WARPS * 32, 0, c->stream>>>(m)));
		if (c->st.max_degree > 32) KEV(OGB_KC_MARK2, c->stream, (k_mark_fast<2><<<grid_for(c, (const void *)k_mark_fast<2>, OGB_WARPS * 32), OGB_WARPS * 32, 0, c->stream>>>(m)));
		c->launches += c->st.max_degree > 32 ? 2 : 1;
		KEV(OGB_KC_MARKANY, c->stream, (k_mark_any<<<grid_for(c, (const void *)k_mark_any, OGB_WARPS * 32), OGB_WARPS * 32, 0, c->stream>>>(m)));
		CUDA_TRY(cudaGetLastError());
		c->launches++;
		if (c->st.max_degree * 2 <= OGB_SETCAP) break;
		OGB_TRY(ctr_fetch(c));
		if (c->h_ctr[CTR_SCRATCH_FAIL] == 0) break;
		u64 need = c->h_ctr[CTR_SCRATCH_CURSOR] + 1024;
		OGB_TRY(c->scratch_keys.ensure(need));
	}
	CUDA_TRY(cudaEventRecord(c->ev[EV_MARK1], c->stream));
	if (G > 1) {
		const int ke = kev_begin(c, OGB_KC_EXCH_BITS, c->stream);
		NCCL_TRY(g_nccl.AllGather(c->ebits.p + per * c->rank, c->ebits.p, per, NCCL_UINT32, c->comm, c->stream));
		if (more_need) NCCL_TRY(g_nccl.AllGather(c->ebits.p + nrows + obit_words * c->rank, c->ebits.p + nrows, obit_words, NCCL_UINT32, c->comm, c->stream));
		kev_end(c, ke, c->stream);
	}

	const int ke_keep = kev_begin(c, OGB_KC_KEEP, c->stream);
	if (nloc) k_keep<<<(nloc + 255) / 256, 256, 0, c->stream>>>(m, c->surv.p);
	k_keep_big<<<c->sm_count, 256, 0, c->stream>>>(m);
	kev_end(c, ke_keep, c->stream);
	const int ke_emit = kev_begin(c, OGB_KC_EMIT, c->stream);
	CUDA_TRY(cudaGetLastError());
	c->launches += 2;
	OGB_TRY(exclusive_scan(c, c->cnt.p, nloc, c->pos.p, c->d_tot + 1));
	if (G == 1) {
		OGB_TRY(c->fin.ensure(std::max<u64>(exact_edges, 1)));
		if (nloc) k_emit_small<<<(nloc + 255) / 256, 256, 0, c->stream>>>(c->surv.p, c->cnt.p, c->cntc.p, c->pos.p, c->fin.p, lo, hi, 0);
		k_emit<false><<<g_emit, OGB_WARPS * 32, 0, c->stream>>>(c->slots_e.p, c->ext.p, c->deg.p, c->cntc.p, c->pos.p, c->fin.p, lo, hi, cap_now, 0, OGB_SURV);
		CUDA_TRY(cudaGetLastError());
		kev_end(c, ke_emit, c->stream);
		c->launches += 2;
		u64 tot = 0;
		CUDA_TRY(cudaMemcpyAsync(&tot, c->d_tot + 1, sizeof(u64), cudaMemcpyDeviceToHost, c->stream));
		OGB_TRY(ctr_fetch(c));
		c->n_final = tot; c->fin_own_off = 0; c->fin_own_cnt = tot;
	} else {
		std::vector<u64> fin_cnt(G, 0), all(G, 0);
		CUDA_TRY(cudaMemcpyAsync(c->d_xchg + c->rank, c->d_tot + 1, sizeof(u64), cudaMemcpyDeviceToDevice, c->stream));
		NCCL_TRY(g_nccl.AllGather(c->d_xchg + c->rank, c->d_xchg, 1, NCCL_UINT64, c->comm, c->stream));
		CUDA_TRY(cudaMemcpyAsync(fin_cnt.data(), c->d_xchg, (size_t)G * sizeof(u64), cudaMemcpyDeviceToHost, c->stream));
		CUDA_TRY(cudaStreamSynchronize(c->stream));
		u64 stride = 0, total = 0;
		for (int r = 0; r < G; r++) { stride = std::max(stride, fin_cnt[r]); total += fin_cnt[r]; }
		stride = (stride + 63) & ~63ull;
		c->n_final = total; c->fin_own_off = 0; for (int r = 0; r < c->rank; r++) c->fin_own_off += fin_cnt[r]; c->fin_own_cnt = fin_cnt[c->rank];
		OGB_TRY(c->fin_stage.ensure(std::max<u64>(stride * G, 1)));
		OGB_TRY(c->fin.ensure(std::max<u64>(total, 1)));
		if (nloc) k_emit_small<<<(nloc + 255) / 256, 256, 0, c->stream>>>(c->surv.p, c->cnt.p, c->cntc.p, c->pos.p, c->fin_stage.p, lo, hi, stride * c->rank);
		k_emit<false><<<g_emit, OGB_WARPS * 32, 0, c->stream>>>(c->slots_e.p, c->ext.p, c->deg.p, c->cntc.p, c->pos.p, c->fin_stage.p, lo, hi, cap_now, stride * c->rank, OGB_SURV);
		CUDA_TRY(cudaGetLastError());
		kev_end(c, ke_emit, c->stream);
		c->launches += 2;
		const int ke_fin = kev_begin(c, OGB_KC_EXCH_FINAL, c->stream);
		OGB_TRY(gather_segments(c, c->fin_stage, stride, fin_cnt, c->fin.p));
		kev_end(c, ke_fin, c->stream);
		NCCL_TRY(g_nccl.AllReduce(c->d_ctr + CTR_NODES_FINAL, c->d_xchg + XCHG_SCRATCH + 2, 1, NCCL_UINT64, 0 , c->comm, c->stream));
		OGB_TRY(ctr_fetch(c));
		CUDA_TRY(cudaMemcpyAsync(&c->h_ctr[CTR_NODES_FINAL], c->d_xchg + XCHG_SCRATCH + 2, sizeof(u64), cudaMemcpyDeviceToHost, c->stream));
		CUDA_TRY(cudaStreamSynchronize(c->stream));
	}
	CUDA_TRY(cudaEventRecord(c->ev[EV_RED1], c->stream));
	CUDA_TRY(cudaStreamSynchronize(c->stream));
	kev_collect(c);
	if (c->h_ctr[CTR_ASYMMETRIC]) { ogb_set_error("ogb_build_graph: %llu edges without a twin (internal error)", (unsigned long long)c->h_ctr[CTR_ASYMMETRIC]); return OGB_E_STATE; }
	{
		u32 want = (u32)std::min<u64>(256, std::max<u64>(32, (c->st.max_degree * 5 / 4 + 7) / 8 * 8));
		if (want < c->slot_cap) c->slot_cap = want;
	}
	c->st.pivot_entries = c->h_ctr[CTR_PIVOT_ENTRIES];
	c->st.active_pivots = c->h_ctr[CTR_ACTIVE_PIVOTS];
	c->st.edges_final = c->n_final;
	c->st.nodes_final = c->h_ctr[CTR_NODES_FINAL];
	c->st.ms_overlap = ev_ms(c, EV_OVL0, EV_OVL1);
	c->st.ms_scan_kernel = ev_ms(c, EV_K3A, EV_K3B);
	{
		float sum = 0;
		for (u32 i = 0; i < c->n_pk; i++) { float ms = 0; if (cudaEventElapsedTime(&ms, c->ev_pk[2 * i], c->ev_pk[2 * i + 1]) == cudaSuccess) sum += ms; else cudaGetLastError(); }
		c->st.ms_probe_launch = c->n_pk ? sum / c->n_pk : 0;
		float wsum = 0;
		if (c->partitioned)
			for (u32 i = 0; i < c->n_pk; i++) { float ms = 0; if (cudaEventElapsedTime(&ms, c->ev_pk[2 * i], c->ev_pm[i]) == cudaSuccess) wsum += ms; else cudaGetLastError(); }
		c->st.ms_window_launch = c->n_pk ? wsum / c->n_pk : 0;
// ... 447 lines not shown
```

### metagenomics_b200/csrc/ogb_kernels.cuh

```cuda
#pragma once
#include <cstdint>
#include <cuda_runtime.h>

typedef unsigned long long u64;
typedef unsigned int u32;

#define OGB_SLOTS 10
#define OGB_BWORDS 16
#define OGB_WARPS 8
#ifndef OGB_PROBE_MINBLOCKS
#define OGB_PROBE_MINBLOCKS 6
#endif
#ifndef OGB_VERIFY_MINBLOCKS
#define OGB_VERIFY_MINBLOCKS 6
#endif
#define OGB_SETCAP 512

enum { MODE_OVERLAP = 0, MODE_CONTAIN = 1 };

enum {
	CTR_EDGE_CURSOR = 0, CTR_OVERFLOW, CTR_PROBES, CTR_SECTORS, CTR_CANDIDATES, CTR_CONTAIN_HITS,
	CTR_PIVOT_ENTRIES, CTR_ACTIVE_PIVOTS, CTR_MAX_DEGREE, CTR_N_CONTAINED, CTR_NODES_FINAL,
	CTR_ASYMMETRIC, CTR_SCRATCH_CURSOR, CTR_SCRATCH_FAIL, CTR_CAND_MAX, CTR_BIG_NODES, CTR_EXT_CURSOR, CTR_PQ_OVERFLOW,
	CTR_TABLE_FULL, CTR_MORE_CURSOR, CTR_MORE_NEED, CTR_BIGREC_CURSOR, CTR_HROW_CURSOR, CTR_COUNT
};

struct ReadStore {
	const u64 *words;
	const u64 *meta;
	u32 n;
	u32 uniform_len;
	u32 uniform_pw;
};

struct Table {
	u32 *slots;
	u32 *summary;
	u32 nb;
	u32 nparts;
	u32 part_buckets;
	u32 sub;
	u32 my_rank;
	u32 h;
	u64 *ctr;
};

__device__ __forceinline__ u32 padded_words(u32 L) { return ((L + 63) >> 6) << 1; }

__device__ __forceinline__ void read_geom(const ReadStore &R, u32 idx, u64 &off, u32 &L)
{
	if (R.uniform_len) { L = R.uniform_len; off = (u64)idx * (2 * R.uniform_pw); }
	else { u64 m = __ldg(R.meta + idx); L = (u32)(m & 0xFFFF); off = m >> 16; }
}

__device__ __forceinline__ u64 ld_na(const u64 *p)
{
	u64 v;
	asm volatile("ld.global.nc.L1::no_allocate.u64 %0, [%1];" : "=l"(v) : "l"(p));
	return v;
}
__device__ __forceinline__ u32 ld_na32(const u32 *p)
{
	u32 v;
	asm volatile("ld.global.nc.L1::no_allocate.u32 %0, [%1];" : "=r"(v) : "l"(p));
	return v;
}
struct LdShared { static __device__ __forceinline__ u64 ld(const u64 *p) { return *p; } };
struct LdGlobal { static __device__ __forceinline__ u64 ld(const u64 *p) { return __ldg(p); } };
struct LdStream { static __device__ __forceinline__ u64 ld(const u64 *p) { return ld_na(p); } };

__device__ __forceinline__ u64 funnel(u64 a, u64 b, u32 sh)
{
	const u32 a1 = (u32)(a >> 32), a0 = (u32)a, b1 = (u32)(b >> 32), b0 = (u32)b;
	const bool hi = sh >= 32;
	const u32 x2 = hi ? a0 : a1, x1 = hi ? b1 : a0, x0 = hi ? b0 : b1;
	return ((u64)__funnelshift_l(x1, x2, sh) << 32) | __funnelshift_l(x0, x1, sh);
}

template <class LD> __device__ __forceinline__ u64 extract32(const u64 *__restrict__ w, u32 p)
{
	u32 wi = p >> 5, sh = (p & 31) << 1;
	return funnel(LD::ld(w + wi), LD::ld(w + wi + 1), sh);
}

__device__ __forceinline__ u64 mix64(u64 acc, u64 x)
{
	acc ^= x;
	acc *= 0xff51afd7ed558ccdULL;
	acc ^= acc >> 33;
	return acc;
}

__device__ __forceinline__ u64 hash2(u64 k0, u64 k1)
{
	u64 acc = 0x9E3779B97F4A7C15ULL;
	acc += (u64)(u32)(k0 >> 32) * 0xD6E8FEB86659FD93ULL;
	acc += (u64)(u32)k0 * 0xA0761D6478BD642FULL;
	acc += (u64)(u32)(k1 >> 32) * 0xE7037ED1A0B428DBULL;
	acc += (u64)(u32)k1 * 0x8EBC6AF09C88C6E3ULL;
	return acc;
}

template <class LD> __device__ __forceinline__ u64 key_hash(const u64 *__restrict__ w, u32 p, u32 h, u32 &lead)
{
	const u32 wi = p >> 5, sh = (p & 31) << 1;
	const u64 a = LD::ld(w + wi), b = LD::ld(w + wi + 1);
	u64 k0 = funnel(a, b, sh);
	if (h <= 32) { k0 &= ~0ULL << (64 - 2 * h); lead = (u32)(k0 >> 32); return hash2(k0, 0); }
	lead = (u32)(k0 >> 32);
	const u64 c = LD::ld(w + wi + 2);
	u64 k1 = funnel(b, c, sh);
	if (h <= 64) return hash2(k0, k1 & (~0ULL << (128 - 2 * h)));
	u64 acc = hash2(k0, k1);
	u32 rem = h - 64;
	p += 64;
	for (; rem > 32; rem -= 32, p += 32) acc = mix64(acc, extract32<LD>(w, p));
	return mix64(acc, extract32<LD>(w, p) & (~0ULL << (64 - 2 * rem)));
}
template <class LD> __device__ __forceinline__ u32 key_lead(const u64 *__restrict__ w, u32 p, u32 h)
{
	u64 k0 = extract32<LD>(w, p);
	if (h < 32) k0 &= ~0ULL << (64 - 2 * h);
	return (u32)(k0 >> 32);
}

__device__ __forceinline__ u32 hash_fp(u64 hash) { u32 f = (u32)hash & 0xFFFFu; return f ? f : 1u; }
#define OGB_SPILLED 0x80000000u
__device__ __forceinline__ u32 summary_bits(u32 fp) { return (1u << min(fp & 31u, 30u)) | (1u << min((fp >> 5) & 31u, 30u)); }

__device__ __forceinline__ u32 partition_of(u32 lead, const Table &T) { return T.nparts == 1 ? 0 : __umulhi(lead * 0x9E3779B1u, T.nparts); }
__device__ __forceinline__ u32 bucket_of(u64 hash, u32 lead, const Table &T, u32 &part)
{
	part = partition_of(lead, T);
	return part * T.part_buckets + __umulhi((u32)(hash >> 32), T.part_buckets);
}
__device__ __forceinline__ u32 next_bucket(u32 b, u32 pend, const Table &T) { return b + 1 == pend ? pend - T.part_buckets : b + 1; }

template <class LDS, class LDT>
__device__ __forceinline__ bool region_equal(const u64 *__restrict__ s, u32 a, const u64 *__restrict__ t, u32 b, u32 len)
{
	const u32 sa = (a & 31) << 1, sb = (b & 31) << 1;
	const u64 *ws = s + (a >> 5), *wt = t + (b >> 5);
	const u64 *es = s + ((a + len - 1) >> 5), *et = t + ((b + len - 1) >> 5);
	u64 s0 = LDS::ld(ws), t0 = LDT::ld(wt), diff = 0;
	u32 k = 0;
	for (; k + 32 <= len; k += 32) {
		++ws; ++wt;
		const u64 s1 = ws <= es ? LDS::ld(ws) : 0, t1 = wt <= et ? LDT::ld(wt) : 0;
		diff |= funnel(s0, s1, sa) ^ funnel(t0, t1, sb);
		s0 = s1; t0 = t1;
	}
	const u32 rem = len - k;
	if (rem) {
		++ws; ++wt;
		const u64 s1 = ws <= es ? LDS::ld(ws) : 0, t1 = wt <= et ? LDT::ld(wt) : 0;
		diff |= (funnel(s0, s1, sa) ^ funnel(t0, t1, sb)) & (~0ULL << (64 - 2 * rem));
	}
	return diff == 0;
}

template <class LDP, class LDQ>
__device__ __forceinline__ bool region_equal_aligned(const u64 *__restrict__ p, u32 pa, const u64 *__restrict__ q, u32 len)
{
	const u32 sh = (pa & 31) << 1;
	const u64 *wp = p + (pa >> 5), *ep = p + ((pa + len - 1) >> 5);
	u64 p0 = LDP::ld(wp), diff = 0;
	u32 k = 0;
	for (; k + 32 <= len; k += 32) {
		++wp;
		const u64 p1 = wp <= ep ? LDP::ld(wp) : 0;
		diff |= funnel(p0, p1, sh) ^ LDQ::ld(q + (k >> 5));
		p0 = p1;
	}
	const u32 rem = len - k;
	if (rem) {
		++wp;
		const u64 p1 = wp <= ep ? LDP::ld(wp) : 0;
// ... 246 lines not shown
{
	const u32 u = blockIdx.x * blockDim.x + threadIdx.x;
	if (u >= nu) return;
	freq[u] = (u + 1 < nu ? ustart[u + 1] : n) - ustart[u];
	const u64 *row = rows + (u64)usrc[u] * W;
	u64 *dst = words + woff[u];
	for (u32 k = 0; k < unw[u]; k++) dst[k] = row[k];
}

__global__ void k_hash_insert(ReadStore R, Table T)
{
	u64 tid = (u64)blockIdx.x * blockDim.x + threadIdx.x;
	if (tid >= (u64)R.n * 4) return;
	u32 idx = (u32)(tid >> 2), o = (u32)(tid & 3);
	u64 off; u32 L;
	read_geom(R, idx, off, L);
	const u64 *w = R.words + off + (o >> 1) * padded_words(L);
	u32 p = (o & 1) ? L - T.h : 0;
	if (T.nparts > T.sub && partition_of(key_lead<LdGlobal>(w, p, T.h), T) / T.sub != T.my_rank) return;
	u32 lead;
	u64 hash = key_hash<LdGlobal>(w, p, T.h, lead);
	const u32 fp = hash_fp(hash), val = ((idx + 1) << 2) | o;
	u32 part;
	u32 b = bucket_of(hash, lead, T, part);
	const u32 pend = (part + 1) * T.part_buckets;
	for (u32 steps = 0;; steps++) {
		if (steps >= T.part_buckets) { atomicMax(T.ctr + CTR_TABLE_FULL, 1ull); return; }
		u32 *w = T.slots + (u64)b * OGB_BWORDS;
		u32 cur[12];
		#pragma unroll
		for (int q = 0; q < 12; q += 4)
			asm volatile("ld.global.cg.v4.u32 {%0,%1,%2,%3}, [%4];" : "=r"(cur[q]), "=r"(cur[q + 1]), "=r"(cur[q + 2]), "=r"(cur[q + 3]) : "l"(w + 4 + q) : "memory");
		int s = OGB_SLOTS;
		#pragma unroll
		for (int q = OGB_SLOTS - 1; q >= 0; q--) s = cur[1 + q] == 0 ? q : s;
		bool done = false;
		for (; s < OGB_SLOTS && !done; s++) done = atomicCAS(w + 5 + s, 0u, val) == 0;
		if (done) { atomicOr(w + ((s - 1) >> 1), fp << (16 * ((s - 1) & 1))); if (T.summary) atomicOr(T.summary + b, summary_bits(fp)); break; }
		if (T.summary) atomicOr(T.summary + b, OGB_SPILLED);
		b = next_bucket(b, pend, T);
	}
}

struct KeyQueue {
	u32 *b, *f, *v;
	u64 *cursor;
	u64 cap;
	u32 nparts;
	u32 first, count;
};
#define OGB_KPT 4
__global__ void __launch_bounds__(256, 6) k_key_part(ReadStore R, Table T, KeyQueue Q)
{
	__shared__ u32 s_cnt[64];
	__shared__ u64 s_base[64];
	const u64 total = (u64)R.n * 4;
	const u32 tile_keys = 256 * OGB_KPT;
	const u64 tiles = (total + tile_keys - 1) / tile_keys;
	for (u64 tile = blockIdx.x; tile < tiles; tile += gridDim.x) {
		if (threadIdx.x < Q.nparts) s_cnt[threadIdx.x] = 0;
		__syncthreads();
		u32 eb[OGB_KPT], ef[OGB_KPT], ev[OGB_KPT], ep[OGB_KPT];
		#pragma unroll
		for (int r = 0; r < OGB_KPT; r++) {
			const u64 x = tile * tile_keys + r * 256 + threadIdx.x;
			ep[r] = 0xFFFFFFFFu; eb[r] = ef[r] = ev[r] = 0;
			if (x >= total) continue;
			const u32 idx = (u32)(x >> 2), o = (u32)(x & 3);
			u64 off; u32 L;
			read_geom(R, idx, off, L);
			const u64 *w = R.words + off + (o >> 1) * padded_words(L);
			const u32 p = (o & 1) ? L - T.h : 0;
			if (T.nparts > T.sub && partition_of(key_lead<LdGlobal>(w, p, T.h), T) / T.sub != T.my_rank) continue;
			u32 lead;
			const u64 hash = key_hash<LdGlobal>(w, p, T.h, lead);
			u32 part;
			eb[r] = bucket_of(hash, lead, T, part);
			ef[r] = hash_fp(hash); ev[r] = ((idx + 1) << 2) | o;
			ep[r] = (part << 16) | atomicAdd(&s_cnt[part], 1u);
		}
		__syncthreads();
		if (threadIdx.x < Q.nparts) s_base[threadIdx.x] = s_cnt[threadIdx.x] ? atomicAdd(Q.cursor + threadIdx.x, (u64)s_cnt[threadIdx.x]) : 0;
		__syncthreads();
		#pragma unroll
		for (int r = 0; r < OGB_KPT; r++)
			if (ep[r] != 0xFFFFFFFFu) {
				const u32 part = ep[r] >> 16;
				const u64 at = s_base[part] + (ep[r] & 0xFFFFu);
				if (at < Q.cap) { const u64 i = (part - Q.first) * Q.cap + at; Q.b[i] = eb[r]; Q.f[i] = ef[r]; Q.v[i] = ev[r]; }
			}
		__syncthreads();
	}
}
__device__ __forceinline__ void insert_record(const Table &T, u32 b, u32 fp, u32 val)
{
	const u32 part = b / T.part_buckets, pend = (part + 1) * T.part_buckets;
	for (u32 steps = 0;; steps++) {
		if (steps >= T.part_buckets) { atomicMax(T.ctr + CTR_TABLE_FULL, 1ull); return; }
		u32 *w = T.slots + (u64)b * OGB_BWORDS;
		u32 cur[12];
		#pragma unroll
		for (int q = 0; q < 12; q += 4)
			asm volatile("ld.global.cg.v4.u32 {%0,%1,%2,%3}, [%4];" : "=r"(cur[q]), "=r"(cur[q + 1]), "=r"(cur[q + 2]), "=r"(cur[q + 3]) : "l"(w + 4 + q) : "memory");
		int s = OGB_SLOTS;
		#pragma unroll
		for (int q = OGB_SLOTS - 1; q >= 0; q--) s = cur[1 + q] == 0 ? q : s;
		bool done = false;
		for (; s < OGB_SLOTS && !done; s++) done = atomicCAS(w + 5 + s, 0u, val) == 0;
		if (done) { atomicOr(w + ((s - 1) >> 1), fp << (16 * ((s - 1) & 1))); if (T.summary) atomicOr(T.summary + b, summary_bits(fp)); return; }
		if (T.summary) atomicOr(T.summary + b, OGB_SPILLED);
		b = next_bucket(b, pend, T);
	}
}
__global__ void __launch_bounds__(256, 6) k_insert_parts(Table T, KeyQueue Q)
{
	const u64 g = (u64)blockIdx.x * blockDim.x + threadIdx.x, nthreads = (u64)gridDim.x * blockDim.x;
	for (u32 part = Q.first; part < Q.first + Q.count; part++) {
		const u64 n = min(Q.cursor[part], Q.cap), base = (part - Q.first) * Q.cap;
		if (Q.cursor[part] > Q.cap && g == 0) atomicMax(T.ctr + CTR_TABLE_FULL, 2ull);
		for (u64 i = g; i < n; i += nthreads) insert_record(T, Q.b[base + i], Q.f[base + i], Q.v[base + i]);
	}
}

__device__ __forceinline__ void load_bucket(const u32 *__restrict__ slots, u32 b, u32 (&w)[OGB_BWORDS])
{
	const u32 *p = slots + (u64)b * OGB_BWORDS;
	u64 x[8];
	asm volatile("ld.global.nc.L1::no_allocate.v4.u64 {%0,%1,%2,%3}, [%4];" : "=l"(x[0]), "=l"(x[1]), "=l"(x[2]), "=l"(x[3]) : "l"(p));
	asm volatile("ld.global.nc.L1::no_allocate.v4.u64 {%0,%1,%2,%3}, [%4];" : "=l"(x[4]), "=l"(x[5]), "=l"(x[6]), "=l"(x[7]) : "l"(p + 8));
	#pragma unroll
	for (int i = 0; i < 8; i++) { w[2 * i] = (u32)x[i]; w[2 * i + 1] = (u32)(x[i] >> 32); }
}

__device__ __forceinline__ u32 match_bucket(const u32 (&w)[OGB_BWORDS], u32 fp)
{
	const u32 splat = fp | (fp << 16);
	u32 z[5], any = 0;
	#pragma unroll
	for (int i = 0; i < 5; i++) { const u32 x = w[i] ^ splat; z[i] = (x - 0x00010001u) & ~x & 0x80008000u; any |= z[i]; }
	if (any == 0) return 0;
	u32 mm = 0;
	#pragma unroll
	for (int i = 0; i < 5; i++) mm |= (((z[i] >> 15) & 1) | ((z[i] >> 30) & 2)) << (2 * i);
	return mm;
}
__device__ __forceinline__ u32 bucket_value(const u32 (&w)[OGB_BWORDS], int k)
{
	u32 v = w[5];
	#pragma unroll
	for (int q = 1; q < OGB_SLOTS; q++) v = (k == q) ? w[5 + q] : v;
	return v;
}

#define OGB_QCHUNK 128
#define OGB_NOCAND 0xFFFFFFFFu

struct ScanArgs {
	ReadStore R;
	Table T;
	u32 lo, hi;
	const u32 *contained;
	u32 *cand_q;
	u64 *cand_v;
	u64 cand_cap;
	u64 *cand_cursor;
	u64 *sup;
	u64 *slots_e;
	u32 slot_lo;
	u32 cap;
	u32 *deg;
	u32 *ov_q;
	u64 *ov_e;
	u64 ov_cap;
	u64 *ctr;
	u32 prefetch;
};

__device__ __forceinline__ void prefetch_l2(const void *p) { asm volatile("prefetch.global.L2 [%0];" ::"l"(p)); }

struct QueueCursor { u64 qbase; u32 qused, qsize; };

__device__ __forceinline__ void queue_pad(const ScanArgs &A, const QueueCursor &Q, u32 lane)
{
	for (u32 i = Q.qused + lane; i < Q.qsize; i += 32) if (Q.qbase + i < A.cand_cap) A.cand_q[Q.qbase + i] = OGB_NOCAND;
}

__device__ __forceinline__ void append_matches(const ScanArgs &A, QueueCursor &Q, u32 lane, u32 mm, const u32 (&w)[OGB_BWORDS], u32 qi, u64 tag)
{
	const u32 cnt = __popc(mm);
	u32 inc = cnt;
	#pragma unroll
	for (int d = 1; d < 32; d <<= 1) { const u32 t = __shfl_up_sync(0xFFFFFFFFu, inc, d); if (lane >= (u32)d) inc += t; }
	const u32 total = __shfl_sync(0xFFFFFFFFu, inc, 31);
	if (Q.qused + total > Q.qsize) {
		queue_pad(A, Q, lane);
		Q.qsize = total > OGB_QCHUNK ? (total + 31) & ~31u : OGB_QCHUNK;
		if (lane == 0) Q.qbase = atomicAdd(A.cand_cursor, (u64)Q.qsize);
		Q.qbase = __shfl_sync(0xFFFFFFFFu, Q.qbase, 0);
		Q.qused = 0;
	}
	u64 at = Q.qbase + Q.qused + (inc - cnt);
	for (; mm; mm &= mm - 1, at++) {
		const u32 v = bucket_value(w, __ffs(mm) - 1);
		if (at < A.cand_cap) { A.cand_q[at] = qi; A.cand_v[at] = tag | v; }
		if (A.prefetch) {
			const u32 ri = (v >> 2) - 1;
			if (A.R.uniform_len) prefetch_l2(A.R.words + (u64)ri * (2 * A.R.uniform_pw) + ((v >> 1) & 1) * A.R.uniform_pw);
			else prefetch_l2(A.R.meta + ri);
		}
	}
	Q.qused += total;
}

#define OGB_PENDQ 64
struct PendQueue {
	u32 b[OGB_WARPS][OGB_PENDQ];
	u32 f[OGB_WARPS][OGB_PENDQ];
	u32 q[OGB_WARPS][OGB_PENDQ];
};

__device__ __forceinline__ void probe_buckets(const ScanArgs &A, QueueCursor &Q, u32 lane, bool active, u32 b, u32 fj, u32 qi, u64 &c_sectors)
{
	const u32 fp = fj & 0xFFFFu;
	const u64 tag = (u64)(fj >> 16) << 32;
	u32 pend = 0, steps = 0;
	while (__any_sync(0xFFFFFFFFu, active)) {
		u32 w[OGB_BWORDS];
		u32 mm = 0;
		if (active) {
			load_bucket(A.T.slots, b, w);
			c_sectors++;
			mm = match_bucket(w, fp);
			active = w[5 + OGB_SLOTS - 1] != 0 && ++steps < A.T.part_buckets;
			if (active) {
				if (pend == 0) pend = (b / A.T.part_buckets + 1) * A.T.part_buckets;
				b = next_bucket(b, pend, A.T);
			}
		}
		if (__any_sync(0xFFFFFFFFu, mm != 0)) append_matches(A, Q, lane, mm, w, qi, tag);
	}
}

__device__ __forceinline__ void pend_push(const ScanArgs &A, PendQueue &P, u32 wib, u32 &plen, QueueCursor &Q, u32 lane, bool pass, u32 b, u32 fj, u32 qi, u64 &c_sectors)
{
	const u32 bal = __ballot_sync(0xFFFFFFFFu, pass);
	if (pass) {
		const u32 at = plen + __popc(bal & ((1u << lane) - 1));
		P.b[wib][at] = b; P.f[wib][at] = fj; P.q[wib][at] = qi;
	}
	plen += __popc(bal);
	__syncwarp();
	if (plen >= 32) {
		plen -= 32;
		const u32 pb = P.b[wib][plen + lane], pf = P.f[wib][plen + lane], pq = P.q[wib][plen + lane];
		__syncwarp();
		probe_buckets(A, Q, lane, true, pb, pf, pq, c_sectors);
	}
}
__device__ __forceinline__ void pend_drain(const ScanArgs &A, PendQueue &P, u32 wib, u32 plen, QueueCursor &Q, u32 lane, u64 &c_sectors)
{
	if (plen == 0) return;
	const bool act = lane < plen;
	const u32 pb = act ? P.b[wib][lane] : 0, pf = act ? P.f[wib][lane] : 0, pq = act ? P.q[wib][lane] : 0;
	probe_buckets(A, Q, lane, act, pb, pf, pq, c_sectors);
}

__device__ __forceinline__ bool window_key(const ScanArgs &A, const u64 *__restrict__ s, u32 j, u32 &b, u32 &fj, u32 &part)
{
	u32 lead;
	const u64 hash = key_hash<LdGlobal>(s, j, A.T.h, lead);
	b = bucket_of(hash, lead, A.T, part);
	const u32 fp = hash_fp(hash);
	fj = fp | (j << 16);
	if (!A.T.summary) return true;
	const u32 sm = ld_na32(A.T.summary + b), need = summary_bits(fp);
	return (sm & need) == need || (sm & OGB_SPILLED);
}

template <int MODE>
__global__ void __launch_bounds__(256, OGB_PROBE_MINBLOCKS) k_probe(ScanArgs A)
{
	__shared__ PendQueue P;
	const u32 lane = threadIdx.x & 31, wib = threadIdx.x >> 5;
	const u32 gw = (blockIdx.x * blockDim.x + threadIdx.x) >> 5, nwarps = (gridDim.x * blockDim.x) >> 5;
	const u32 h = A.T.h;
	u64 c_probes = 0, c_sectors = 0;
	u32 plen = 0;
	QueueCursor Q = {0, 0, 0};

	for (u32 qi = A.lo + gw; qi < A.hi; qi += nwarps) {
		if (MODE == MODE_OVERLAP && A.contained && ((__ldg(A.contained + (qi >> 5)) >> (qi & 31)) & 1)) continue;
		u64 off; u32 L1;
		read_geom(A.R, qi, off, L1);
		const u64 *s = A.R.words + off;
		const u32 nwin = L1 - h - 1;
		c_probes += nwin;
		for (u32 jb = 1; jb <= nwin; jb += 32) {
			const u32 j = jb + lane;
			u32 b = 0, fj = 0, part;
			const bool pass = j <= nwin && window_key(A, s, j, b, fj, part);
			pend_push(A, P, wib, plen, Q, lane, pass, b, fj, qi, c_sectors);
		}
	}
	pend_drain(A, P, wib, plen, Q, lane, c_sectors);
	queue_pad(A, Q, lane);
	for (int d = 16; d > 0; d >>= 1) c_sectors += __shfl_down_sync(0xFFFFFFFFu, c_sectors, d);
	if (lane == 0) { atomicAdd(A.ctr + CTR_PROBES, c_probes); atomicAdd(A.ctr + CTR_SECTORS, c_sectors); }
}

template <int MODE>
__global__ void __launch_bounds__(256, OGB_PROBE_MINBLOCKS) k_probe_uniform(ScanArgs A, u32 nwin, u64 div_magic)
{
	__shared__ PendQueue P;
	const u32 lane = threadIdx.x & 31, wib = threadIdx.x >> 5;
	const u32 total = (A.hi - A.lo) * nwin;
	const u32 rounds = (total + 31) >> 5;
	const u32 gw = (blockIdx.x * blockDim.x + threadIdx.x) >> 5, nwarps = (gridDim.x * blockDim.x) >> 5;
	const u32 stride = 2 * A.R.uniform_pw;
	u64 c_sectors = 0;
	u32 plen = 0;
	QueueCursor Q = {0, 0, 0};

	for (u32 rd = gw; rd < rounds; rd += nwarps) {
		const u32 x = rd * 32 + lane;
		const u32 qr = nwin == 1 ? x : (u32)__umul64hi(div_magic, (u64)x);
		const u32 j = x - qr * nwin + 1, qi = A.lo + qr;
		u32 b = 0, fj = 0, part;
		const bool pass = x < total && window_key(A, A.R.words + (u64)qi * stride, j, b, fj, part);
		pend_push(A, P, wib, plen, Q, lane, pass, b, fj, qi, c_sectors);
	}
	pend_drain(A, P, wib, plen, Q, lane, c_sectors);
	queue_pad(A, Q, lane);
	for (int d = 16; d > 0; d >>= 1) c_sectors += __shfl_down_sync(0xFFFFFFFFu, c_sectors, d);
	if (lane == 0) atomicAdd(A.ctr + CTR_SECTORS, c_sectors);
	if (blockIdx.x == 0 && threadIdx.x == 0) atomicAdd(A.ctr + CTR_PROBES, (u64)total);
}

#define OGB_MAXPART 64
#ifndef OGB_WPT
#define OGB_WPT 4
#endif
struct PartQueue {
	u32 *b, *f, *q;
	u64 *cursor;
	u64 cap;
	u32 nparts;
};

template <int MODE, bool UNIFORM>
__global__ void __launch_bounds__(256, 6) k_window_part(ScanArgs A, u32 nwin, u64 div_magic, PartQueue PQ)
{
	__shared__ u32 s_cnt[OGB_MAXPART];
	__shared__ u64 s_base[OGB_MAXPART];
	__shared__ u32 s_valid;
	const u32 total = (A.hi - A.lo) * nwin;
	const u32 stride = 2 * A.R.uniform_pw;
	const u32 tile_windows = 256 * OGB_WPT;
	const u32 tiles = (total + tile_windows - 1) / tile_windows;
	const u32 h = A.T.h;
	u32 c_valid = 0;
	if (threadIdx.x == 0) s_valid = 0;
	for (u32 tile = blockIdx.x; tile < tiles; tile += gridDim.x) {
		if (threadIdx.x < PQ.nparts) s_cnt[threadIdx.x] = 0;
		__syncthreads();
		u32 eb[OGB_WPT], ef[OGB_WPT], eq[OGB_WPT], ep[OGB_WPT];
		#pragma unroll
		for (int r = 0; r < OGB_WPT; r++) {
			const u32 x = tile * tile_windows + r * 256 + threadIdx.x;
			const u32 qr = nwin == 1 ? x : (u32)__umul64hi(div_magic, (u64)x);
			const u32 j = x - qr * nwin + 1;
			eq[r] = A.lo + qr; eb[r] = 0; ef[r] = 0;
			u32 part = 0;
			bool valid = x < total;
			const u64 *s = nullptr;
			if (UNIFORM) s = A.R.words + (u64)eq[r] * stride;
			else if (valid) {
				u64 off; u32 L1;
				read_geom(A.R, eq[r], off, L1);
				s = A.R.words + off;
				valid = j <= L1 - h - 1;
				if (MODE == MODE_OVERLAP && valid && A.contained) valid = !((__ldg(A.contained + (eq[r] >> 5)) >> (eq[r] & 31)) & 1);
				c_valid += valid;
			}
			const bool pass = valid && window_key(A, s, j, eb[r], ef[r], part);
			ep[r] = pass ? (part << 16) | atomicAdd(&s_cnt[part], 1u) : 0xFFFFFFFFu;
		}
		__syncthreads();
		if (threadIdx.x < PQ.nparts) s_base[threadIdx.x] = s_cnt[threadIdx.x] ? atomicAdd(PQ.cursor + threadIdx.x, (u64)s_cnt[threadIdx.x]) : 0;
		__syncthreads();
		#pragma unroll
		for (int r = 0; r < OGB_WPT; r++)
			if (ep[r] != 0xFFFFFFFFu) {
				const u32 part = ep[r] >> 16;
				const u64 at = s_base[part] + (ep[r] & 0xFFFFu);
				if (at < PQ.cap) { const u64 i = part * PQ.cap + at; PQ.b[i] = eb[r]; PQ.f[i] = ef[r]; PQ.q[i] = eq[r]; }
			}
		__syncthreads();
	}
	if (UNIFORM) { if (blockIdx.x == 0 && threadIdx.x == 0) atomicAdd(A.ctr + CTR_PROBES, (u64)total); }
	else {
		c_valid = __reduce_add_sync(0xFFFFFFFFu, c_valid);
		if ((threadIdx.x & 31) == 0 && c_valid) atomicAdd(&s_valid, c_valid);
		__syncthreads();
		if (threadIdx.x == 0 && s_valid) atomicAdd(A.ctr + CTR_PROBES, (u64)s_valid);
	}
}

template <int MODE>
__device__ __forceinline__ void probe_parts_body(const ScanArgs &A, const PartQueue &PQ, u64 gw, u64 nwarps, u32 lane)
{
	u64 c_sectors = 0;
	QueueCursor Q = {0, 0, 0};
	for (u32 part = 0; part < PQ.nparts; part++) {
		const u64 filled = PQ.cursor[part];
		if (filled > PQ.cap && gw == 0 && lane == 0) atomicMax(A.ctr + CTR_PQ_OVERFLOW, filled);
		const u64 n = min(filled, PQ.cap), base = part * PQ.cap;
		for (u64 i0 = gw * 32; i0 < n; i0 += nwarps * 32) {
			const u64 i = i0 + lane;
			const bool act = i < n;
			const u32 pb = act ? PQ.b[base + i] : 0, pf = act ? PQ.f[base + i] : 0, pq = act ? PQ.q[base + i] : 0;
			probe_buckets(A, Q, lane, act, pb, pf, pq, c_sectors);
		}
	}
	queue_pad(A, Q, lane);
	for (int d = 16; d > 0; d >>= 1) c_sectors += __shfl_down_sync(0xFFFFFFFFu, c_sectors, d);
	if (lane == 0) atomicAdd(A.ctr + CTR_SECTORS, c_sectors);
}
template <int MODE>
__global__ void __launch_bounds__(256, OGB_PROBE_MINBLOCKS) k_probe_parts(ScanArgs A, PartQueue PQ)
{
	probe_parts_body<MODE>(A, PQ, (blockIdx.x * (u64)blockDim.x + threadIdx.x) >> 5, (gridDim.x * (u64)blockDim.x) >> 5, threadIdx.x & 31);
}

template <int MODE>
__device__ __forceinline__ void verify_body(const ScanArgs &A, u64 first, u64 stride, bool announce)
{
	const u64 total = min(*A.cand_cursor, A.cand_cap);
	if (announce) atomicMax(A.ctr + CTR_CAND_MAX, *A.cand_cursor);
	const u32 h = A.T.h, lane = threadIdx.x & 31, lt = (1u << lane) - 1;
	u32 c_cand = 0, c_hits = 0;
	for (u64 c0 = first; c0 < total; c0 += stride) {
		const u64 c = c0 + lane;
		bool ok = false;
		u32 qi = c < total ? A.cand_q[c] : OGB_NOCAND, ri = 0, o = 0, L1 = 0, L2 = 0, orient = 0, offset = 0;
		if (qi != OGB_NOCAND) {
			const u64 cv = A.cand_v[c];
			const u32 j = (u32)(cv >> 32), val = (u32)cv;
			if (val != 0) {
				c_cand++;
				u64 off, roff;
				read_geom(A.R, qi, off, L1);
				const u64 *s = A.R.words + off;
				ri = (val >> 2) - 1; o = val & 3;
				read_geom(A.R, ri, roff, L2);
				const u64 *t = A.R.words + roff + (o >> 1) * padded_words(L2);
				if (MODE == MODE_CONTAIN) {
					if (L1 > L2) {
						u32 a = 0; bool fits;
						if ((o & 1) == 0) { fits = L1 - j >= L2; a = j; }
						else { fits = j >= L2 - h; a = j - (L2 - h); }
						if (fits && region_equal_aligned<LdGlobal, LdGlobal>(s, a, t, L2)) {
							atomicMax(A.sup + ri, ((u64)L1 << 32) | (u64)(0xFFFFFFFFu - qi));
							c_hits++;
						}
					}
				} else if (!(A.contained && ((__ldg(A.contained + (ri >> 5)) >> (ri & 31)) & 1))) {
					u32 pa, len; bool fits;
					const u64 *pp, *qq;
					if ((o & 1) == 0) {
						fits = L1 - j < L2;
						pp = s; pa = j; qq = t; len = L1 - j;
						orient = o == 0 ? 3 : 2;
						offset = j;
					} else {
						fits = L2 - h >= j;
						pp = t; pa = L2 - h - j; qq = s; len = h + j;
						orient = o == 1 ? 0 : 1;
						offset = L1 - h - j;
					}
					if (!fits) ok = false;
					else if (A.R.uniform_pw == 4) ok = suffix_equals_prefix<4>(pp, pa, qq, len);
					else if (A.R.uniform_pw == 6) ok = suffix_equals_prefix<6>(pp, pa, qq, len);
					else ok = region_equal_aligned<LdGlobal, LdGlobal>(pp, pa, qq, len);
				}
			}
		}
		if (MODE == MODE_OVERLAP) {
			const u32 ne = ok ? (ri == qi ? 2u : 1u) : 0u;
			const u32 grp = __match_any_sync(0xFFFFFFFFu, ok ? qi : (0x80000000u | lane));
			const int leader = __ffs(grp) - 1;
			const u32 b1 = __ballot_sync(0xFFFFFFFFu, ne >= 1), b2 = __ballot_sync(0xFFFFFFFFu, ne == 2);
			const u32 all = __popc(grp & b1) + __popc(grp & b2);
			const u32 before = __popc(grp & b1 & lt) + __popc(grp & b2 & lt);
			u32 base = 0;
			if (ok && (int)lane == leader) base = atomicAdd(A.deg + qi, all);
			base = __shfl_sync(0xFFFFFFFFu, base, leader);
			if (ok) {
				const u64 e0 = make_edge(offset & 0xFFFF, ri + 1, orient), e1 = make_edge(offset & 0xFFFF, ri + 1, twin_orient(orient));
				for (u32 q = 0; q < ne; q++) {
					const u64 e = q ? e1 : e0;
					const u32 pos = base + before + q;
					if (pos < A.cap) A.slots_e[(u64)(qi - A.slot_lo) * A.cap + pos] = e;
					else {
						if (pos == A.cap) atomicAdd(A.ctr + CTR_BIG_NODES, 1ull);
						const u64 ov = atomicAdd(A.ctr + CTR_OVERFLOW, 1ull);
						if (ov < A.ov_cap) { A.ov_q[ov] = qi; A.ov_e[ov] = e; }
					}
				}
			}
		}
	}
	for (int d = 16; d > 0; d >>= 1) { c_cand += __shfl_down_sync(0xFFFFFFFFu, c_cand, d); c_hits += __shfl_down_sync(0xFFFFFFFFu, c_hits, d); }
	if (lane == 0) {
		if (c_cand) atomicAdd(A.ctr + CTR_CANDIDATES, (u64)c_cand);
		if (MODE == MODE_CONTAIN && c_hits) atomicAdd(A.ctr + CTR_CONTAIN_HITS, (u64)c_hits);
	}
}
template <int MODE>
__global__ void __launch_bounds__(256, OGB_VERIFY_MINBLOCKS) k_verify(ScanArgs A)
{
	verify_body<MODE>(A, (u64)blockIdx.x * blockDim.x + (threadIdx.x - (threadIdx.x & 31)), (u64)gridDim.x * blockDim.x, blockIdx.x == 0 && threadIdx.x == 0);
}
template <int MODE>
__global__ void __launch_bounds__(256, OGB_PROBE_MINBLOCKS) k_probe_verify(ScanArgs AP, PartQueue PQ, ScanArgs AV)
{
	const u32 lane = threadIdx.x & 31, wib = threadIdx.x >> 5;
	if (wib < 4) probe_parts_body<MODE>(AP, PQ, (u64)blockIdx.x * 4 + wib, (u64)gridDim.x * 4, lane);
	else verify_body<MODE>(AV, (u64)blockIdx.x * 128 + (wib - 4) * 32, (u64)gridDim.x * 128, blockIdx.x == 0 && threadIdx.x == 128);
}

#define OGB_KEEP 2ull
#define OGB_ROW_W 32
#define OGB_ROW_E 30
#define OGB_SURV 4

struct GraphView {
	u64 *slots;
	const u32 *deg;
	u64 *ext;
	u32 lo, cap;
	u32 *rows;
	u32 *more;
	u32 *ebits;
	u64 more_stride;
	u64 nrows;
	u64 per_magic;
	u32 my_rank;
};

__device__ __forceinline__ u32 row_entry(u64 e) { return (edge_dst(e) << 1) | ((edge_orient(e) >> 1) & 1); }
__device__ __forceinline__ u32 rank_of(const GraphView &G, u32 vidx) { return G.per_magic ? (u32)__umul64hi(G.per_magic, (u64)vidx) : 0u; }
__device__ __forceinline__ u64 entry_bit(const GraphView &G, u32 vidx, u32 pos)
{
	if (pos < OGB_ROW_E) return (u64)vidx * 32 + pos + 1;
	const u32 ovf = __ldg(G.rows + (u64)vidx * OGB_ROW_W + 1);
	return G.nrows * 32 + (u64)rank_of(G, vidx) * G.more_stride + ovf + (pos - OGB_ROW_E) + 1;
}

#define OGB_HROW_W 34
template <bool HEAVY>
__global__ void __launch_bounds__(256) k_rows_finish(GraphView G, u32 lo, u32 hi, u32 *__restrict__ more_own, u64 more_cap, u64 *ctr,
                                                     u32 *__restrict__ hrows, u64 hrows_cap)
{
	const u32 lane = threadIdx.x & 31;
	const u32 gw = (blockIdx.x * blockDim.x + threadIdx.x) >> 5, nwarps = (gridDim.x * blockDim.x) >> 5;
	for (u32 u0 = lo + gw * 32; u0 < hi; u0 += nwarps * 32) {
		const u32 mine = u0 + lane;
		u32 dm = mine < hi ? G.deg[mine] : 0;
		const bool heavy = dm > G.cap;
		if (heavy != HEAVY) dm = HEAVY ? 0 : 0xFFFFFFFFu;
		const u32 need = dm != 0xFFFFFFFFu && dm > OGB_ROW_E ? dm - OGB_ROW_E : 0;
		u32 inc = need;
		#pragma unroll
		for (int s = 1; s < 32; s <<= 1) { const u32 t = __shfl_up_sync(0xFFFFFFFFu, inc, s); if (lane >= (u32)s) inc += t; }
		const u32 total = __shfl_sync(0xFFFFFFFFu, inc, 31);
		u64 base = 0;
		if (total) {
			if (lane == 31) base = atomicAdd(ctr + CTR_MORE_CURSOR, (u64)total);
			base = __shfl_sync(0xFFFFFFFFu, base, 31);
		}
		const u64 offm = base + inc - need;
		const u32 cnt = min(32u, hi - u0);
		for (u32 j = 0; j < cnt; j++) {
			const u32 u = u0 + j;
			const u32 d = __shfl_sync(0xFFFFFFFFu, dm, j);
			const u64 off = __shfl_sync(0xFFFFFFFFu, offm, j);
			u32 *row = G.rows + (u64)u * OGB_ROW_W;
			if (d == 0xFFFFFFFFu) continue;
			if (d == 0) { if (!HEAVY && lane == 0) row[0] = 0; continue; }
			const u64 *own = G.slots + (u64)(u - G.lo) * G.cap;
			if (HEAVY) own = G.ext + own[0];
			u32 wv = lane == 0 ? d : (u32)off;
			if (lane >= 2) wv = lane - 2 < d ? row_entry(own[lane - 2]) : 0;
			row[lane] = wv;
			if (HEAVY && hrows) {
				u64 at = 0;
				if (lane == 0) at = atomicAdd(ctr + CTR_HROW_CURSOR, 1ull);
				at = __shfl_sync(0xFFFFFFFFu, at, 0);
				if (at < hrows_cap) { u32 *r = hrows + at * OGB_HROW_W; if (lane == 0) { r[0] = u; r[1] = 0; } r[2 + lane] = wv; }
			}
			if (d > OGB_ROW_E && off + (d - OGB_ROW_E) <= more_cap)
				for (u32 k = OGB_ROW_E + lane; k < d; k += 32) more_own[off + k - OGB_ROW_E] = row_entry(own[k]);
		}
	}
}
__global__ void __launch_bounds__(256) k_scatter_hrows(const u32 *__restrict__ hrows, u64 stride, const u64 *__restrict__ counts, u32 nranks, u32 my_rank, u32 *__restrict__ rows)
{
	const u32 lane = threadIdx.x & 31;
	const u64 gw = ((u64)blockIdx.x * blockDim.x + threadIdx.x) >> 5, nwarps = ((u64)gridDim.x * blockDim.x) >> 5;
	for (u32 r = 0; r < nranks; r++) {
		if (r == my_rank) continue;
		for (u64 i = gw; i < counts[r]; i += nwarps) {
			const u32 *rec = hrows + (r * stride + i) * OGB_HROW_W;
			rows[(u64)rec[0] * OGB_ROW_W + lane] = rec[2 + lane];
		}
	}
}

__global__ void __launch_bounds__(256) k_heavy_move(u64 *__restrict__ slots, const u32 *__restrict__ deg, u32 lo, u32 hi, u32 cap,
                                                   u64 *__restrict__ ext, u64 ext_cap, u32 *__restrict__ fill, u64 *ctr)
{
	const u32 u = lo + blockIdx.x * blockDim.x + threadIdx.x;
	if (u >= hi) return;
	const u32 d = deg[u];
	if (d <= cap) return;
	const u64 off = atomicAdd(ctr + CTR_EXT_CURSOR, (u64)d);
	if (off + d > ext_cap) { atomicAdd(ctr + CTR_SCRATCH_FAIL, 1ull); return; }
	u64 *s = slots + (u64)(u - lo) * cap;
	for (u32 k = 0; k < cap; k++) ext[off + k] = s[k];
	fill[u - lo] = cap;
	s[0] = off;
}
__global__ void __launch_bounds__(256) k_heavy_place(const u32 *__restrict__ ov_q, const u64 *__restrict__ ov_e, u64 n_over, const u64 *__restrict__ slots,
                                                    u32 lo, u32 cap, u64 *__restrict__ ext, u32 *__restrict__ fill)
{
	const u64 i = (u64)blockIdx.x * blockDim.x + threadIdx.x;
	if (i >= n_over) return;
	const u32 u = ov_q[i];
	const u64 off = slots[(u64)(u - lo) * cap];
	ext[off + atomicAdd(fill + (u - lo), 1u)] = ov_e[i];
}

__global__ void k_contained_bitmap(const u64 *__restrict__ sup, u32 n, u32 *__restrict__ bitmap, u64 *ctr)
{
	u32 idx = blockIdx.x * blockDim.x + threadIdx.x;
	bool c = idx < n && sup[idx] != 0;
	u32 bal = __ballot_sync(0xFFFFFFFFu, c);
	if ((threadIdx.x & 31) == 0 && idx < n) {
		bitmap[idx >> 5] = bal;
		if (bal) atomicAdd(ctr + CTR_N_CONTAINED, (u64)__popc(bal));
	}
}

struct MarkArgs {
	GraphView G;
	u32 hi;
	u32 *cntc;
	u64 *cand;
	u64 *big;
	u64 big_cap;
	u32 *cnt;
	u32 *scratch_keys;
	u64 scratch_cap;
	u64 *ctr;
};

#define OGB_SET_ELIM 0x80000000u
#define OGB_SET_KEY 0x3FFFFFFFu
__device__ __forceinline__ u32 set_hash(u32 key, u32 capmask) { return (key * 2654435761u) >> 7 & capmask; }

__device__ __forceinline__ u32 set_insert(u32 *keys, u32 capmask, u32 key)
{
	u32 s = set_hash(key, capmask);
	for (;;) {
		u32 cur = atomicCAS(keys + s, 0u, key);
		if (cur == 0 || (cur & OGB_SET_KEY) == key) return s;
		s = (s + 1) & capmask;
	}
}
__device__ __forceinline__ int set_find(const u32 *keys, u32 capmask, u32 key)
{
	u32 s = set_hash(key, capmask);
	for (;;) {
// ... 689 lines not shown
```

Before: 334.2 million.

## Bin candidate queue by partner read range to localize verify gathers

Splits the candidate queue into up to 16 bins keyed by partner read id, so the store is divided into roughly 256 MiB slices. Probe warps append candidates through per-bin 32-entry pieces tracked in shared memory, and verify walks the bins one after another so partner reads are gathered from an L2-sized working set. It also removes the experimental fused probe+verify path. The cost is more warp-level match/shuffle work per append, extra padding entries and less capacity per bin.

Result: slower. 279.3 million (median of 6 runs) (-16.4%).

```diff
diff --git a/include/ogb.h b/include/ogb.h
--- a/include/ogb.h
+++ b/include/ogb.h
@@ -89,6 +89,7 @@
 	float ms_window_launch;
 	float ms_kernel[OGB_KC_COUNT];
 	uint32_t n_kernel[OGB_KC_COUNT];
+	uint32_t partner_bins;
 } ogb_stats;
 
 int ogb_version(void);
diff --git a/metagenomics_b200/_lib.py b/metagenomics_b200/_lib.py
--- a/metagenomics_b200/_lib.py
+++ b/metagenomics_b200/_lib.py
@@ -26,7 +26,7 @@
         ("kernel_launches", C.c_uint32), ("probe_launches", C.c_uint32), ("hash_partitions", C.c_uint32), ("hash_build_attempts", C.c_uint32)] + [(n, C.c_float) for n in (
             "ms_pack", "ms_hash_build", "ms_contain", "ms_overlap", "ms_exchange_pre", "ms_mark", "ms_reduce",
             "ms_total", "ms_scan_kernel", "ms_probe_launch", "ms_window_launch")] + [
-        ("ms_kernel", C.c_float * 20), ("n_kernel", C.c_uint32 * 20)]
+        ("ms_kernel", C.c_float * 20), ("n_kernel", C.c_uint32 * 20), ("partner_bins", C.c_uint32)]
 
     KERNEL_CLASSES = ("hash_insert", "window_part", "probe_parts", "verify", "rows_finish", "mark_fast1", "mark_fast2", "mark_any", "keep", "emit",
                       "contain_window", "contain_probe", "contain_verify", "exch_index", "exch_rows", "exch_bits", "exch_final", "probe_verify")
diff --git a/metagenomics_b200/csrc/ogb_device.cu b/metagenomics_b200/csrc/ogb_device.cu
--- a/metagenomics_b200/csrc/ogb_device.cu
+++ b/metagenomics_b200/csrc/ogb_device.cu
@@ -141,6 +141,8 @@
 	Pool<u32> cand_q, fill, ov_q;
 	Pool<u64> cand_v, ov_e;
 	u64 cand_cap = 0;
+	u32 nbins = 1, bin_mul = 0;
+	u64 store_words = 0;
 	Pool<u32> pq_b, pq_f, pq_q;
 	u64 *d_pq_cursor = nullptr;
 	bool partitioned = false, part_chunk_set = false;
@@ -220,6 +222,8 @@
 	}
 	c->n_kev = 0;
 }
+#define OGB_PARTNER_BIN_TARGET (256ull << 20)
+
 #define KEV(cls, stream, launch) do { const int kev_i_ = kev_begin(c, cls, stream); launch; kev_end(c, kev_i_, stream); } while (0)
 
 static int fetch_words_cb(ogb_dataset *ds);
@@ -274,7 +278,7 @@
 	for (int i = 0; i < 64; i++) CUDA_TRY(cudaEventCreate(&c->ev_pm[i]));
 	CUDA_TRY(cudaMalloc((void **)&c->d_ctr, CTR_COUNT * sizeof(u64)));
 	CUDA_TRY(cudaMalloc((void **)&c->d_tot, 2 * sizeof(u64)));
-	CUDA_TRY(cudaMalloc((void **)&c->d_cursor, 2 * sizeof(u64)));
+	CUDA_TRY(cudaMalloc((void **)&c->d_cursor, 2 * OGB_MAXBINS * sizeof(u64)));
 	CUDA_TRY(cudaMalloc((void **)&c->d_pq_cursor, OGB_MAXPART * sizeof(u64)));
 	CUDA_TRY(cudaMalloc((void **)&c->d_xchg, XCHG_WORDS * sizeof(u64)));
 	CUDA_TRY(cudaMemset(c->d_xchg, 0, XCHG_WORDS * sizeof(u64)));
@@ -413,6 +417,7 @@
 static int upload_common(ogb_context *c, u64 total_words, const std::vector<u64> &meta_host)
 {
 	OGB_TRY(c->words.ensure(total_words + 8));
+	c->store_words = total_words;
 	CUDA_TRY(cudaMemsetAsync(c->words.p + total_words, 0, 8 * sizeof(u64), c->stream));
 	if (!meta_host.empty()) {
 		OGB_TRY(c->meta.ensure(meta_host.size()));
@@ -946,6 +951,7 @@
 	a.R = c->rs(); a.T = c->tb(); a.lo = lo; a.hi = hi;
 	a.contained = c->any_contained ? c->contained.p : nullptr;
 	a.cand_q = c->cand_q.p; a.cand_v = c->cand_v.p; a.cand_cap = c->cand_cap; a.cand_cursor = c->d_cursor;
+	a.nbins = c->nbins; a.bin_mul = c->bin_mul;
 	a.sup = c->sup.p; a.slots_e = c->slots_e.p; a.slot_lo = lo; a.cap = c->slot_cap; a.deg = c->deg.p;
 	a.ov_q = c->ov_q.p; a.ov_e = c->ov_e.p; a.ov_cap = c->ov_q.cap; a.ctr = c->d_ctr; a.prefetch = 1;
 	return a;
@@ -1044,8 +1050,17 @@
 	} else
 	if (c->chunk_reads > (1u << 16)) c->chunk_reads = 1u << 16;
 	{
-		const u64 want = part_mode ? std::max<u64>(32ull << 20, (u64)c->chunk_reads * 40) : 8ull << 20;
-		if (c->cand_cap < want) { OGB_TRY(c->cand_q.ensure(2 * want)); OGB_TRY(c->cand_v.ensure(2 * want)); c->cand_cap = want; }
+		u64 target = OGB_PARTNER_BIN_TARGET;
+		const char *e = getenv("OGB_PARTNER_BIN_BYTES");
+		if (e && atoll(e) >= 1) target = (u64)atoll(e);
+		const u64 bytes = c->store_words * sizeof(u64);
+		c->nbins = (u32)std::max<u64>(1, std::min<u64>(OGB_MAXBINS, std::min<u64>(c->n, (bytes + target - 1) / target)));
+		c->bin_mul = c->nbins == 1 ? 0 : (u32)std::min<u64>(0xFFFFFFFFull, (((u64)c->nbins << 32) + c->n - 1) / c->n);
+		u64 want = part_mode ? std::max<u64>(32ull << 20, (u64)c->chunk_reads * 40) : 8ull << 20;
+		const char *ee = getenv("OGB_CAND_ENTRIES");
+		if (ee && atoll(ee) >= 1024) want = (u64)atoll(ee);
+		c->cand_cap = (want + want / 4) / c->nbins;
+		OGB_TRY(c->cand_q.ensure(2 * c->nbins * c->cand_cap)); OGB_TRY(c->cand_v.ensure(2 * c->nbins * c->cand_cap));
 	}
 	int gp = grid_for(c, (const void *)k_probe<MODE>, 256), gv = grid_for(c, (const void *)k_verify<MODE>, 256);
 	int gu = grid_for(c, (const void *)k_probe_uniform<MODE>, 256);
@@ -1064,71 +1079,17 @@
 	const u32 n_chunks = (u32)(((xchg ? per_rank : (u64)(hi - lo)) + c->chunk_reads - 1) / c->chunk_reads);
 	const GraphView gv_rows = graph_view(c, lo);
 	const int g_rows = grid_for(c, (const void *)k_rows_finish<false>, 256);
-	const bool fused = part_mode && getenv("OGB_FUSED") && atoi(getenv("OGB_FUSED")) == 1;
-	bool have_prev = false;
-	ScanArgs a_prev = a;
-	u32 prev_i = 0;
-	auto finish_chunk = [&](const ScanArgs &av, u32 ci, cudaStream_t after) -> int {
-		if (MODE != MODE_OVERLAP) return OGB_OK;
-		CUDA_TRY(cudaEventRecord(c->ev_rows[ci & 1], after));
-		CUDA_TRY(cudaStreamWaitEvent(c->xs, c->ev_rows[ci & 1], 0));
-		KEV(OGB_KC_ROWS, c->xs, (k_rows_finish<false><<<std::min<int>(g_rows, (int)((av.hi - av.lo + 255) / 256)), 256, 0, c->xs>>>(gv_rows, av.lo, av.hi, c->more_own.p, c->more_cap, c->d_ctr, nullptr, 0)));
-		c->launches++;
-		if (xchg) {
-			const int ke = kev_begin(c, OGB_KC_EXCH_ROWS, c->xs);
-			OGB_TRY(exchange_chunk_rows(c, ci, c->xs));
-			kev_end(c, ke, c->xs);
-		}
-		return OGB_OK;
-	};
-	auto flush_prev = [&]() -> int {
-		if (!have_prev) return OGB_OK;
-		KEV(MODE == MODE_OVERLAP ? OGB_KC_VERIFY : OGB_KC_CONTAIN_VERIFY, c->stream, (k_verify<MODE><<<gv, 256, 0, c->stream>>>(a_prev)));
-		c->launches++;
-		have_prev = false;
-		return finish_chunk(a_prev, prev_i, c->stream);
-	};
 	for (; i < n_chunks; i++) {
 		const u64 b0 = (u64)lo + (u64)i * c->chunk_reads;
 		const int q = i & 1;
 		if (b0 >= hi) {
-			if (fused) OGB_TRY(flush_prev());
 			if (xchg) { const int ke = kev_begin(c, OGB_KC_EXCH_ROWS, c->xs); OGB_TRY(exchange_chunk_rows(c, i, c->xs)); kev_end(c, ke, c->xs); }
 			continue;
 		}
-		if (fused) {
-			a.lo = (u32)b0; a.hi = (u32)std::min<u64>(hi, b0 + c->chunk_reads);
-			a.cand_q = c->cand_q.p + q * c->cand_cap; a.cand_v = c->cand_v.p + q * c->cand_cap; a.cand_cursor = c->d_cursor + q;
-			a.prefetch = 0;
-			CUDA_TRY(cudaMemsetAsync(a.cand_cursor, 0, sizeof(u64), c->stream));
-			CUDA_TRY(cudaMemsetAsync(c->d_pq_cursor, 0, OGB_MAXPART * sizeof(u64), c->stream));
-			PartQueue pq;
-			pq.b = c->pq_b.p; pq.f = c->pq_f.p; pq.q = c->pq_q.p; pq.cursor = c->d_pq_cursor; pq.cap = c->pq_cap; pq.nparts = c->nparts;
-			const u32 nreads = a.hi - a.lo;
-			const u64 tiles = ((u64)nreads * nwin_u + 256 * OGB_WPT - 1) / (256 * OGB_WPT);
-			const bool uni = c->uniform_len && !a.contained;
-			const int gw = grid_for(c, uni ? (const void *)k_window_part<MODE, true> : (const void *)k_window_part<MODE, false>, 256);
-			const int kc = MODE == MODE_OVERLAP ? 0 : OGB_KC_CONTAIN_WINDOW - OGB_KC_WINDOW;
-			const bool timed = MODE == MODE_OVERLAP && i < 64;
-			if (timed) CUDA_TRY(cudaEventRecord(c->ev_pk[2 * i], c->stream));
-			if (uni) KEV(OGB_KC_WINDOW + kc, c->stream, (k_window_part<MODE, true><<<(unsigned)std::min<u64>(gw, tiles), 256, 0, c->stream>>>(a, nwin_u, ~0ull / nwin_u + 1, pq)));
-			else KEV(OGB_KC_WINDOW + kc, c->stream, (k_window_part<MODE, false><<<(unsigned)std::min<u64>(gw, tiles), 256, 0, c->stream>>>(a, nwin_u, ~0ull / nwin_u + 1, pq)));
-			if (timed) CUDA_TRY(cudaEventRecord(c->ev_pm[i], c->stream));
-			if (have_prev) {
-				KEV(MODE == MODE_OVERLAP ? OGB_KC_PROBE_VERIFY : OGB_KC_CONTAIN_PROBE, c->stream,
-				    (k_probe_verify<MODE><<<grid_for(c, (const void *)k_probe_verify<MODE>, 256), 256, 0, c->stream>>>(a, pq, a_prev)));
-				OGB_TRY(finish_chunk(a_prev, prev_i, c->stream));
-			} else
-				KEV(OGB_KC_PROBE + kc, c->stream, (k_probe_parts<MODE><<<grid_for(c, (const void *)k_probe_parts<MODE>, 256), 256, 0, c->stream>>>(a, pq)));
-			if (timed) { CUDA_TRY(cudaEventRecord(c->ev_pk[2 * i + 1], c->stream)); c->n_pk = i + 1; }
-			c->launches += 2;
-			have_prev = true; a_prev = a; prev_i = i;
-			continue;
-		}
 		a.lo = (u32)b0; a.hi = (u32)std::min<u64>(hi, b0 + c->chunk_reads);
-		a.cand_q = c->cand_q.p + q * c->cand_cap; a.cand_v = c->cand_v.p + q * c->cand_cap; a.cand_cursor = c->d_cursor + q;
+		a.cand_q = c->cand_q.p + q * c->nbins * c->cand_cap; a.cand_v = c->cand_v.p + q * c->nbins * c->cand_cap; a.cand_cursor = c->d_cursor + q * OGB_MAXBINS;
 		if (overlap_streams && i >= 2) CUDA_TRY(cudaStreamWaitEvent(c->stream, c->ev_verify[q], 0));
-		CUDA_TRY(cudaMemsetAsync(a.cand_cursor, 0, sizeof(u64), c->stream));
+		CUDA_TRY(cudaMemsetAsync(a.cand_cursor, 0, c->nbins * sizeof(u64), c->stream));
 		const u32 warps = a.hi - a.lo;
 		const bool timed = MODE == MODE_OVERLAP && i < 64;
 		if (timed) CUDA_TRY(cudaEventRecord(c->ev_pk[2 * i], c->stream));
@@ -1172,8 +1133,7 @@
 		if (overlap_streams) CUDA_TRY(cudaEventRecord(c->ev_verify[q], sv));
 		c->launches += 2;
 	}
-	if (fused) OGB_TRY(flush_prev());
-	if (overlap_streams && !fused)
+	if (overlap_streams)
 		for (int q = 0; q < 2 && q < (int)i; q++) CUDA_TRY(cudaStreamWaitEvent(c->stream, c->ev_verify[q], 0));
 	if (MODE == MODE_OVERLAP) { CUDA_TRY(cudaEventRecord(c->ev_xs, c->xs)); CUDA_TRY(cudaStreamWaitEvent(c->stream, c->ev_xs, 0)); }
 	CUDA_TRY(cudaGetLastError());
@@ -1370,6 +1330,12 @@
 	c->st.overlap_probes = c->h_ctr[CTR_PROBES];
 	c->st.probe_sectors = c->h_ctr[CTR_SECTORS];
 	c->st.candidates = c->h_ctr[CTR_CANDIDATES];
+	c->st.partner_bins = c->nbins;
+#ifdef OGB_REPORT_QUEUE_FILL
+	fprintf(stderr, "ogb: partner bins %u, candidate queue entries %llu for %llu candidates (padding %.2f %%)\n", c->nbins,
+	        (unsigned long long)c->h_ctr[CTR_CAND_SLOTS], (unsigned long long)c->h_ctr[CTR_CANDIDATES],
+	        c->h_ctr[CTR_CAND_SLOTS] ? 100.0 * (1.0 - (double)c->h_ctr[CTR_CANDIDATES] / c->h_ctr[CTR_CAND_SLOTS]) : 0.0);
+#endif
 	c->st.edges_pre_local = local_edges;
 	c->st.edges_pre = exact_edges;
 	c->n_pre = exact_edges;
diff --git a/metagenomics_b200/csrc/ogb_kernels.cuh b/metagenomics_b200/csrc/ogb_kernels.cuh
--- a/metagenomics_b200/csrc/ogb_kernels.cuh
+++ b/metagenomics_b200/csrc/ogb_kernels.cuh
@@ -22,7 +22,7 @@
 	CTR_EDGE_CURSOR = 0, CTR_OVERFLOW, CTR_PROBES, CTR_SECTORS, CTR_CANDIDATES, CTR_CONTAIN_HITS,
 	CTR_PIVOT_ENTRIES, CTR_ACTIVE_PIVOTS, CTR_MAX_DEGREE, CTR_N_CONTAINED, CTR_NODES_FINAL,
 	CTR_ASYMMETRIC, CTR_SCRATCH_CURSOR, CTR_SCRATCH_FAIL, CTR_CAND_MAX, CTR_BIG_NODES, CTR_EXT_CURSOR, CTR_PQ_OVERFLOW,
-	CTR_TABLE_FULL, CTR_MORE_CURSOR, CTR_MORE_NEED, CTR_BIGREC_CURSOR, CTR_HROW_CURSOR, CTR_COUNT
+	CTR_TABLE_FULL, CTR_MORE_CURSOR, CTR_MORE_NEED, CTR_BIGREC_CURSOR, CTR_HROW_CURSOR, CTR_CAND_SLOTS, CTR_COUNT
 };
 
 struct ReadStore {
@@ -575,7 +575,8 @@
 	return v;
 }
 
-#define OGB_QCHUNK 128
+#define OGB_QPIECE 32
+#define OGB_MAXBINS 16
 #define OGB_NOCAND 0xFFFFFFFFu
 
 struct ScanArgs {
@@ -587,6 +588,8 @@
 	u64 *cand_v;
 	u64 cand_cap;
 	u64 *cand_cursor;
+	u32 nbins;
+	u32 bin_mul;
 	u64 *sup;
 	u64 *slots_e;
 	u32 slot_lo;
@@ -601,38 +604,62 @@
 
 __device__ __forceinline__ void prefetch_l2(const void *p) { asm volatile("prefetch.global.L2 [%0];" ::"l"(p)); }
 
-struct QueueCursor { u64 qbase; u32 qused, qsize; };
+struct QueueCursor { u64 *nxt; };
+
+__device__ __forceinline__ QueueCursor queue_open(u64 (&s_nxt)[OGB_WARPS][OGB_MAXBINS], u32 wib, u32 lane)
+{
+	if (lane < OGB_MAXBINS) s_nxt[wib][lane] = 0;
+	__syncwarp();
+	return QueueCursor{s_nxt[wib]};
+}
 
 __device__ __forceinline__ void queue_pad(const ScanArgs &A, const QueueCursor &Q, u32 lane)
 {
-	for (u32 i = Q.qused + lane; i < Q.qsize; i += 32) if (Q.qbase + i < A.cand_cap) A.cand_q[Q.qbase + i] = OGB_NOCAND;
+	__syncwarp();
+	for (u32 b = 0; b < A.nbins; b++) {
+		const u64 p = Q.nxt[b];
+		const u32 used = (u32)(p % OGB_QPIECE);
+		if (used == 0) continue;
+		for (u32 i = used + lane; i < OGB_QPIECE; i += 32) {
+			const u64 at = p - used + i;
+			if (at < A.cand_cap) A.cand_q[(u64)b * A.cand_cap + at] = OGB_NOCAND;
+		}
+	}
 }
 
 __device__ __forceinline__ void append_matches(const ScanArgs &A, QueueCursor &Q, u32 lane, u32 mm, const u32 (&w)[OGB_BWORDS], u32 qi, u64 tag)
 {
-	const u32 cnt = __popc(mm);
-	u32 inc = cnt;
-	#pragma unroll
-	for (int d = 1; d < 32; d <<= 1) { const u32 t = __shfl_up_sync(0xFFFFFFFFu, inc, d); if (lane >= (u32)d) inc += t; }
-	const u32 total = __shfl_sync(0xFFFFFFFFu, inc, 31);
-	if (Q.qused + total > Q.qsize) {
-		queue_pad(A, Q, lane);
-		Q.qsize = total > OGB_QCHUNK ? (total + 31) & ~31u : OGB_QCHUNK;
-		if (lane == 0) Q.qbase = atomicAdd(A.cand_cursor, (u64)Q.qsize);
-		Q.qbase = __shfl_sync(0xFFFFFFFFu, Q.qbase, 0);
-		Q.qused = 0;
-	}
-	u64 at = Q.qbase + Q.qused + (inc - cnt);
-	for (; mm; mm &= mm - 1, at++) {
-		const u32 v = bucket_value(w, __ffs(mm) - 1);
-		if (at < A.cand_cap) { A.cand_q[at] = qi; A.cand_v[at] = tag | v; }
-		if (A.prefetch) {
-			const u32 ri = (v >> 2) - 1;
-			if (A.R.uniform_len) prefetch_l2(A.R.words + (u64)ri * (2 * A.R.uniform_pw) + ((v >> 1) & 1) * A.R.uniform_pw);
-			else prefetch_l2(A.R.meta + ri);
-		}
-	}
-	Q.qused += total;
+	const u32 lt = (1u << lane) - 1;
+	for (;;) {
+		u32 v = 0;
+		while (mm && v == 0) { v = bucket_value(w, __ffs(mm) - 1); mm &= mm - 1; }
+		const bool has = v != 0;
+		if (!__any_sync(0xFFFFFFFFu, has)) return;
+		const u32 ri = (v >> 2) - 1;
+		const u32 bin = has ? min(__umulhi(ri, A.bin_mul), A.nbins - 1) : 0;
+		const u32 grp = __match_any_sync(0xFFFFFFFFu, has ? bin : 0x80000000u | lane);
+		const u32 leader = __ffs(grp) - 1, rank = __popc(grp & lt);
+		u64 p = 0, fresh = 0;
+		if (has && lane == leader) {
+			const u32 cnt = __popc(grp);
+			p = Q.nxt[bin];
+			const u32 room = p % OGB_QPIECE ? OGB_QPIECE - (u32)(p % OGB_QPIECE) : 0;
+			if (cnt > room) { fresh = atomicAdd(A.cand_cursor + bin, (u64)OGB_QPIECE); Q.nxt[bin] = fresh + (cnt - room); }
+			else Q.nxt[bin] = p + cnt;
+		}
+		p = __shfl_sync(0xFFFFFFFFu, p, leader);
+		fresh = __shfl_sync(0xFFFFFFFFu, fresh, leader);
+		if (has) {
+			const u64 room = p % OGB_QPIECE ? OGB_QPIECE - p % OGB_QPIECE : 0;
+			const u64 at = rank < room ? p + rank : fresh + (rank - room);
+			if (at < A.cand_cap) { const u64 i = (u64)bin * A.cand_cap + at; A.cand_q[i] = qi; A.cand_v[i] = tag | v; }
+			if (A.prefetch) {
+				if (A.R.uniform_len) prefetch_l2(A.R.words + (u64)ri * (2 * A.R.uniform_pw) + ((v >> 1) & 1) * A.R.uniform_pw);
+				else prefetch_l2(A.R.meta + ri);
+			}
+		}
+		__syncwarp();
+	}
 }
 
 #define OGB_PENDQ 64
@@ -704,12 +731,13 @@
 __global__ void __launch_bounds__(256, OGB_PROBE_MINBLOCKS) k_probe(ScanArgs A)
 {
 	__shared__ PendQueue P;
+	__shared__ u64 s_nxt[OGB_WARPS][OGB_MAXBINS];
 	const u32 lane = threadIdx.x & 31, wib = threadIdx.x >> 5;
 	const u32 gw = (blockIdx.x * blockDim.x + threadIdx.x) >> 5, nwarps = (gridDim.x * blockDim.x) >> 5;
 	const u32 h = A.T.h;
 	u64 c_probes = 0, c_sectors = 0;
 	u32 plen = 0;
-	QueueCursor Q = {0, 0, 0};
+	QueueCursor Q = queue_open(s_nxt, wib, lane);
 
 	for (u32 qi = A.lo + gw; qi < A.hi; qi += nwarps) {
 		if (MODE == MODE_OVERLAP && A.contained && ((__ldg(A.contained + (qi >> 5)) >> (qi & 31)) & 1)) continue;
@@ -735,6 +763,7 @@
 __global__ void __launch_bounds__(256, OGB_PROBE_MINBLOCKS) k_probe_uniform(ScanArgs A, u32 nwin, u64 div_magic)
 {
 	__shared__ PendQueue P;
+	__shared__ u64 s_nxt[OGB_WARPS][OGB_MAXBINS];
 	const u32 lane = threadIdx.x & 31, wib = threadIdx.x >> 5;
 	const u32 total = (A.hi - A.lo) * nwin;
 	const u32 rounds = (total + 31) >> 5;
@@ -742,7 +771,7 @@
 	const u32 stride = 2 * A.R.uniform_pw;
 	u64 c_sectors = 0;
 	u32 plen = 0;
-	QueueCursor Q = {0, 0, 0};
+	QueueCursor Q = queue_open(s_nxt, wib, lane);
 
 	for (u32 rd = gw; rd < rounds; rd += nwarps) {
 		const u32 x = rd * 32 + lane;
@@ -830,10 +859,13 @@
 }
 
 template <int MODE>
-__device__ __forceinline__ void probe_parts_body(const ScanArgs &A, const PartQueue &PQ, u64 gw, u64 nwarps, u32 lane)
-{
+__global__ void __launch_bounds__(256, OGB_PROBE_MINBLOCKS) k_probe_parts(ScanArgs A, PartQueue PQ)
+{
+	__shared__ u64 s_nxt[OGB_WARPS][OGB_MAXBINS];
+	const u32 lane = threadIdx.x & 31;
+	const u64 gw = (blockIdx.x * (u64)blockDim.x + threadIdx.x) >> 5, nwarps = (gridDim.x * (u64)blockDim.x) >> 5;
 	u64 c_sectors = 0;
-	QueueCursor Q = {0, 0, 0};
+	QueueCursor Q = queue_open(s_nxt, threadIdx.x >> 5, lane);
 	for (u32 part = 0; part < PQ.nparts; part++) {
 		const u64 filled = PQ.cursor[part];
 		if (filled > PQ.cap && gw == 0 && lane == 0) atomicMax(A.ctr + CTR_PQ_OVERFLOW, filled);
@@ -849,85 +881,84 @@
 	for (int d = 16; d > 0; d >>= 1) c_sectors += __shfl_down_sync(0xFFFFFFFFu, c_sectors, d);
 	if (lane == 0) atomicAdd(A.ctr + CTR_SECTORS, c_sectors);
 }
+
 template <int MODE>
-__global__ void __launch_bounds__(256, OGB_PROBE_MINBLOCKS) k_probe_parts(ScanArgs A, PartQueue PQ)
-{
-	probe_parts_body<MODE>(A, PQ, (blockIdx.x * (u64)blockDim.x + threadIdx.x) >> 5, (gridDim.x * (u64)blockDim.x) >> 5, threadIdx.x & 31);
-}
-
-template <int MODE>
-__device__ __forceinline__ void verify_body(const ScanArgs &A, u64 first, u64 stride, bool announce)
-{
-	const u64 total = min(*A.cand_cursor, A.cand_cap);
-	if (announce) atomicMax(A.ctr + CTR_CAND_MAX, *A.cand_cursor);
+__global__ void __launch_bounds__(256, OGB_VERIFY_MINBLOCKS) k_verify(ScanArgs A)
+{
+	const u64 first = (u64)blockIdx.x * blockDim.x + (threadIdx.x - (threadIdx.x & 31)), stride = (u64)gridDim.x * blockDim.x;
+	const bool announce = blockIdx.x == 0 && threadIdx.x == 0;
 	const u32 h = A.T.h, lane = threadIdx.x & 31, lt = (1u << lane) - 1;
 	u32 c_cand = 0, c_hits = 0;
-	for (u64 c0 = first; c0 < total; c0 += stride) {
-		const u64 c = c0 + lane;
-		bool ok = false;
-		u32 qi = c < total ? A.cand_q[c] : OGB_NOCAND, ri = 0, o = 0, L1 = 0, L2 = 0, orient = 0, offset = 0;
-		if (qi != OGB_NOCAND) {
-			const u64 cv = A.cand_v[c];
-			const u32 j = (u32)(cv >> 32), val = (u32)cv;
-			if (val != 0) {
-				c_cand++;
-				u64 off, roff;
-				read_geom(A.R, qi, off, L1);
-				const u64 *s = A.R.words + off;
-				ri = (val >> 2) - 1; o = val & 3;
-				read_geom(A.R, ri, roff, L2);
-				const u64 *t = A.R.words + roff + (o >> 1) * padded_words(L2);
-				if (MODE == MODE_CONTAIN) {
-					if (L1 > L2) {
-						u32 a = 0; bool fits;
-						if ((o & 1) == 0) { fits = L1 - j >= L2; a = j; }
-						else { fits = j >= L2 - h; a = j - (L2 - h); }
-						if (fits && region_equal_aligned<LdGlobal, LdGlobal>(s, a, t, L2)) {
-							atomicMax(A.sup + ri, ((u64)L1 << 32) | (u64)(0xFFFFFFFFu - qi));
-							c_hits++;
+	for (u32 bin = 0; bin < A.nbins; bin++) {
+		const u64 filled = A.cand_cursor[bin], total = min(filled, A.cand_cap), rbase = (u64)bin * A.cand_cap;
+		if (announce) { atomicMax(A.ctr + CTR_CAND_MAX, filled); atomicAdd(A.ctr + CTR_CAND_SLOTS, total); }
+		for (u64 c0 = first; c0 < total; c0 += stride) {
+			const u64 c = rbase + c0 + lane;
+			bool ok = false;
+			u32 qi = c0 + lane < total ? A.cand_q[c] : OGB_NOCAND, ri = 0, o = 0, L1 = 0, L2 = 0, orient = 0, offset = 0;
+			if (qi != OGB_NOCAND) {
+				const u64 cv = A.cand_v[c];
+				const u32 j = (u32)(cv >> 32), val = (u32)cv;
+				if (val != 0) {
+					c_cand++;
+					u64 off, roff;
+					read_geom(A.R, qi, off, L1);
+					const u64 *s = A.R.words + off;
+					ri = (val >> 2) - 1; o = val & 3;
+					read_geom(A.R, ri, roff, L2);
+					const u64 *t = A.R.words + roff + (o >> 1) * padded_words(L2);
+					if (MODE == MODE_CONTAIN) {
+						if (L1 > L2) {
+							u32 a = 0; bool fits;
+							if ((o & 1) == 0) { fits = L1 - j >= L2; a = j; }
+							else { fits = j >= L2 - h; a = j - (L2 - h); }
+							if (fits && region_equal_aligned<LdGlobal, LdGlobal>(s, a, t, L2)) {
+								atomicMax(A.sup + ri, ((u64)L1 << 32) | (u64)(0xFFFFFFFFu - qi));
+								c_hits++;
+							}
 						}
+					} else if (!(A.contained && ((__ldg(A.contained + (ri >> 5)) >> (ri & 31)) & 1))) {
+						u32 pa, len; bool fits;
+						const u64 *pp, *qq;
+						if ((o & 1) == 0) {
+							fits = L1 - j < L2;
+							pp = s; pa = j; qq = t; len = L1 - j;
+							orient = o == 0 ? 3 : 2;
+							offset = j;
+						} else {
+							fits = L2 - h >= j;
+							pp = t; pa = L2 - h - j; qq = s; len = h + j;
+							orient = o == 1 ? 0 : 1;
+							offset = L1 - h - j;
+						}
+						if (!fits) ok = false;
+						else if (A.R.uniform_pw == 4) ok = suffix_equals_prefix<4>(pp, pa, qq, len);
+						else if (A.R.uniform_pw == 6) ok = suffix_equals_prefix<6>(pp, pa, qq, len);
+						else ok = region_equal_aligned<LdGlobal, LdGlobal>(pp, pa, qq, len);
 					}
-				} else if (!(A.contained && ((__ldg(A.contained + (ri >> 5)) >> (ri & 31)) & 1))) {
-					u32 pa, len; bool fits;
-					const u64 *pp, *qq;
-					if ((o & 1) == 0) {
-						fits = L1 - j < L2;
-						pp = s; pa = j; qq = t; len = L1 - j;
-						orient = o == 0 ? 3 : 2;
-						offset = j;
-					} else {
-						fits = L2 - h >= j;
-						pp = t; pa = L2 - h - j; qq = s; len = h + j;
-						orient = o == 1 ? 0 : 1;
-						offset = L1 - h - j;
-					}
-					if (!fits) ok = false;
-					else if (A.R.uniform_pw == 4) ok = suffix_equals_prefix<4>(pp, pa, qq, len);
-					else if (A.R.uniform_pw == 6) ok = suffix_equals_prefix<6>(pp, pa, qq, len);
-					else ok = region_equal_aligned<LdGlobal, LdGlobal>(pp, pa, qq, len);
 				}
 			}
-		}
-		if (MODE == MODE_OVERLAP) {
-			const u32 ne = ok ? (ri == qi ? 2u : 1u) : 0u;
-			const u32 grp = __match_any_sync(0xFFFFFFFFu, ok ? qi : (0x80000000u | lane));
-			const int leader = __ffs(grp) - 1;
-			const u32 b1 = __ballot_sync(0xFFFFFFFFu, ne >= 1), b2 = __ballot_sync(0xFFFFFFFFu, ne == 2);
-			const u32 all = __popc(grp & b1) + __popc(grp & b2);
-			const u32 before = __popc(grp & b1 & lt) + __popc(grp & b2 & lt);
-			u32 base = 0;
-			if (ok && (int)lane == leader) base = atomicAdd(A.deg + qi, all);
-			base = __shfl_sync(0xFFFFFFFFu, base, leader);
-			if (ok) {
-				const u64 e0 = make_edge(offset & 0xFFFF, ri + 1, orient), e1 = make_edge(offset & 0xFFFF, ri + 1, twin_orient(orient));
-				for (u32 q = 0; q < ne; q++) {
-					const u64 e = q ? e1 : e0;
-					const u32 pos = base + before + q;
-					if (pos < A.cap) A.slots_e[(u64)(qi - A.slot_lo) * A.cap + pos] = e;
-					else {
-						if (pos == A.cap) atomicAdd(A.ctr + CTR_BIG_NODES, 1ull);
-						const u64 ov = atomicAdd(A.ctr + CTR_OVERFLOW, 1ull);
-						if (ov < A.ov_cap) { A.ov_q[ov] = qi; A.ov_e[ov] = e; }
+			if (MODE == MODE_OVERLAP) {
+				const u32 ne = ok ? (ri == qi ? 2u : 1u) : 0u;
+				const u32 grp = __match_any_sync(0xFFFFFFFFu, ok ? qi : (0x80000000u | lane));
+				const int leader = __ffs(grp) - 1;
+				const u32 b1 = __ballot_sync(0xFFFFFFFFu, ne >= 1), b2 = __ballot_sync(0xFFFFFFFFu, ne == 2);
+				const u32 all = __popc(grp & b1) + __popc(grp & b2);
+				const u32 before = __popc(grp & b1 & lt) + __popc(grp & b2 & lt);
+				u32 base = 0;
+				if (ok && (int)lane == leader) base = atomicAdd(A.deg + qi, all);
+				base = __shfl_sync(0xFFFFFFFFu, base, leader);
+				if (ok) {
+					const u64 e0 = make_edge(offset & 0xFFFF, ri + 1, orient), e1 = make_edge(offset & 0xFFFF, ri + 1, twin_orient(orient));
+					for (u32 q = 0; q < ne; q++) {
+						const u64 e = q ? e1 : e0;
+						const u32 pos = base + before + q;
+						if (pos < A.cap) A.slots_e[(u64)(qi - A.slot_lo) * A.cap + pos] = e;
+						else {
+							if (pos == A.cap) atomicAdd(A.ctr + CTR_BIG_NODES, 1ull);
+							const u64 ov = atomicAdd(A.ctr + CTR_OVERFLOW, 1ull);
+							if (ov < A.ov_cap) { A.ov_q[ov] = qi; A.ov_e[ov] = e; }
+						}
 					}
 				}
 			}
@@ -939,19 +970,6 @@
 		if (MODE == MODE_CONTAIN && c_hits) atomicAdd(A.ctr + CTR_CONTAIN_HITS, (u64)c_hits);
 	}
 }
-template <int MODE>
-__global__ void __launch_bounds__(256, OGB_VERIFY_MINBLOCKS) k_verify(ScanArgs A)
-{
-	verify_body<MODE>(A, (u64)blockIdx.x * blockDim.x + (threadIdx.x - (threadIdx.x & 31)), (u64)gridDim.x * blockDim.x, blockIdx.x == 0 && threadIdx.x == 0);
-}
-template <int MODE>
-__global__ void __launch_bounds__(256, OGB_PROBE_MINBLOCKS) k_probe_verify(ScanArgs AP, PartQueue PQ, ScanArgs AV)
-{
-	const u32 lane = threadIdx.x & 31, wib = threadIdx.x >> 5;
-	if (wib < 4) probe_parts_body<MODE>(AP, PQ, (u64)blockIdx.x * 4 + wib, (u64)gridDim.x * 4, lane);
-	else verify_body<MODE>(AV, (u64)blockIdx.x * 128 + (wib - 4) * 32, (u64)gridDim.x * 128, blockIdx.x == 0 && threadIdx.x == 128);
-}
-
 #define OGB_KEEP 2ull
 #define OGB_ROW_W 32
 #define OGB_ROW_E 30
diff --git a/profiles/gather_sweep.py b/profiles/gather_sweep.py
--- /dev/null
+++ b/profiles/gather_sweep.py
@@ -0,0 +1,27 @@
+import argparse
+import ctypes as C
+import os
+import sys
+
+sys.path.insert(0, os.path.dirname(os.path.dirname(os.path.abspath(__file__))))
+
+
+def main():
+    ap = argparse.ArgumentParser()
+    ap.add_argument("--mib", type=int, nargs="+", default=[64, 128, 256, 512, 1024])
+    ap.add_argument("--bytes", type=int, nargs="+", default=[32, 64])
+    a = ap.parse_args()
+    from metagenomics_b200 import Context
+    from metagenomics_b200._lib import check, lib
+    L = lib()
+    ctx = Context(0)
+    for gb in a.bytes:
+        for mib in a.mib:
+            v = C.c_double()
+            check(L.ogb_gather_ceiling(ctx._h, mib << 20, gb, C.byref(v)))
+            print(f"buffer {mib:5d} MiB  {gb:3d}-byte gathers: {v.value:8.1f} GB/s useful ({v.value / gb:7.1f} G gathers/s)", flush=True)
+    ctx.close()
+
+
+if __name__ == "__main__":
+    main()
diff --git a/profiles/partner_bins_table.py b/profiles/partner_bins_table.py
--- /dev/null
+++ b/profiles/partner_bins_table.py
@@ -0,0 +1,17 @@
+import glob
+import json
+import os
+import sys
+
+d = sys.argv[1] if len(sys.argv) > 1 else "partner_bins_out"
+for p in sorted(glob.glob(os.path.join(d, "c*_*.json"))):
+    try:
+        r = json.loads(open(p).read().strip().splitlines()[-1])
+    except Exception as e:
+        print(f"{os.path.basename(p):22s} no result ({e})")
+        continue
+    k = r.get("kernels", {})
+    row = lambda n: f"{k[n]['ms_per_step']:.3f} ms / {k[n]['launches_per_step']}" if n in k else "-"
+    print(f"{os.path.basename(p):22s} value {r['value'] / 1e6:8.2f} M reads/s  step {r['ms_per_step']:7.3f} ms  parity {r['parity']}"
+          f"  simplify {r.get('simplify', {}).get('parity')}  probe_parts {row('probe_parts')}  verify {row('verify')}"
+          f"  K3 {r['phases_ms']['ms_overlap']:.3f} ms  bins {r.get('stats', {}).get('partner_bins', '-')}")
```
